# rlog58/dags-vae-search

Hardware: AMD Instinct MI355X
Metric: DAGs/sec VAE+predictor train step, n=12 batch 4096 per GPU, at 1 MI355X (higher is better)
Workload: dtype f32 (fwd bf16x6, bwd bf16x3 split products, fp32 accumulate); 1 GPU; synthetic_v12 DAGs (n=12, card=12, N=15 tokens), PACE-VAE train step: pack + fwd + bwd + clip_grad_norm_(1.0) + Adam(1e-4), train mode dropout 0.15; per_gpu_batch=4096, global_batch=4096, waves_per_workgroup=8, parallelism=single

## Files before the change

dags_vae_search_amd/_lib.py:

```python
from __future__ import annotations

import ctypes
import os
from ctypes import (POINTER, Structure, c_char, c_char_p, c_float, c_int, c_int32, c_int64, c_size_t, c_uint32,
                    c_uint64, c_void_p)

_HERE = os.path.dirname(os.path.abspath(__file__))
LIB_NAME = "libdvs_hip.so"

D_MODEL, HEADS, LAYERS, LATENT, FC_HIDDEN, EMB = 64, 8, 3, 32, 32, 32
MAX_TOKENS = 48
TILE_TOKENS = 16
DECODE_STATE_BYTES = 440
CLIP_SCRATCH_FLOATS = 4096
RECORD_BYTES = 96
LOSS_FLOATS = 5
ABI_VERSION = 202
GP_ACQ_MAX_INDUCING = 1023
STRUCT_HASH_INVALID = 0x7FFFFFFFFFFFFFFF
GEN_LABELS_CHOICE, GEN_ACCEPT_ISOLATES, GEN_ACCEPT_NO_CONNECTIVITY, GEN_GROUP_SHIFT = 1, 2, 4, 8
SCORE_TYPES = {"loglik": 0, "aic": 1, "bic": 2, "bde": 3, "bds": 4, "k2": 5, "bdj": 6}


class DvsShape(Structure):
# ... 21 lines not shown
    lib.dvs_record_bytes.argtypes = [P(DvsShape)]
    lib.dvs_pack_features.restype = c_int
    lib.dvs_pack_features.argtypes = [P(DvsShape), c_void_p, c_void_p, c_void_p, c_void_p, c_void_p, c_size_t, c_void_p,
                                      c_void_p]
    lib.dvs_build_records.restype = c_int
    lib.dvs_build_records.argtypes = [P(DvsShape), c_void_p, c_void_p, c_void_p, c_size_t, c_void_p, c_void_p]
    lib.dvs_loss_forward.restype = c_int
    lib.dvs_loss_forward.argtypes = [P(DvsShape), c_void_p, c_size_t, c_void_p, c_int64, c_void_p, c_size_t, c_void_p,
                                     c_void_p, c_void_p, c_void_p, c_void_p, c_void_p]
    lib.dvs_loss_forward_notify.restype = c_int
    lib.dvs_loss_forward_notify.argtypes = [P(DvsShape), c_void_p, c_size_t, c_void_p, c_int64, c_void_p, c_size_t, c_void_p,
                                            c_void_p, c_void_p, c_void_p, c_void_p, c_void_p, ctypes.c_uint32, c_void_p]
    lib.dvs_loss_backward.restype = c_int
    lib.dvs_loss_backward.argtypes = [P(DvsShape), c_void_p, c_size_t, c_void_p, c_int64, c_void_p, c_size_t, c_void_p,
                                      c_void_p, c_void_p]
    lib.dvs_loss_backward_sq.restype = c_int
    lib.dvs_loss_backward_sq.argtypes = [P(DvsShape), c_void_p, c_size_t, c_void_p, c_int64, c_void_p, c_size_t, c_void_p,
                                         c_void_p, c_void_p, c_void_p]
    lib.dvs_encode.restype = c_int
    lib.dvs_encode.argtypes = [P(DvsShape), c_void_p, c_size_t, c_void_p, c_int64, c_void_p, c_size_t, c_void_p, c_void_p,
                               c_void_p]
    lib.dvs_decode.restype = c_int
    lib.dvs_decode.argtypes = [P(DvsShape), c_void_p, c_int64, c_void_p, c_size_t, c_void_p, c_size_t, c_void_p, c_void_p,
                               c_void_p, c_size_t, c_void_p]
    lib.dvs_match_decoded.restype = c_int
    lib.dvs_match_decoded.argtypes = [c_int32, c_int32, c_int32, c_int32, c_int32, c_void_p, c_void_p, c_void_p, c_size_t,
                                      c_int32, c_void_p, c_void_p]
    lib.dvs_decoded_structures.restype = c_int
    lib.dvs_decoded_structures.argtypes = [c_int32, c_int32, c_int32, c_void_p, c_size_t, c_uint64, c_void_p, c_void_p,
                                           c_void_p, c_void_p, c_size_t, c_void_p, c_void_p]
    lib.dvs_structset_filter.restype = c_int
    lib.dvs_structset_filter.argtypes = [c_int32, c_int32, c_void_p, c_void_p, c_void_p, c_size_t, c_void_p, c_int32,
                                         c_void_p, c_void_p, c_size_t, c_void_p, c_void_p]
    lib.dvs_generate_dags.restype = c_int
    lib.dvs_generate_dags.argtypes = [c_int32, c_int32, c_int32, c_int32, c_void_p, c_uint64, c_int64, c_int32, c_int32,
                                      c_void_p, c_void_p, c_size_t, c_void_p, c_void_p]
    lib.dvs_generate_edge_counts.restype = c_int
    lib.dvs_generate_edge_counts.argtypes = [c_int32, c_int32, c_void_p, c_void_p, c_uint64, c_int64, c_void_p, c_void_p]
    lib.dvs_debug_launch.restype = c_int
    lib.dvs_debug_launch.argtypes = [c_size_t, c_void_p]
    lib.dvs_bic_scores.restype = c_int
    lib.dvs_bic_scores.argtypes = [c_int32, c_int32, c_int32, c_void_p, c_void_p, c_void_p, c_void_p, c_void_p, c_void_p,
                                   c_void_p]
    lib.dvs_bn_scores.restype = c_int
    lib.dvs_bn_scores.argtypes = [c_int32, c_int32, c_int32, c_void_p, c_void_p, c_void_p, c_int32, ctypes.c_double, c_void_p,
                                  c_void_p, c_void_p, c_void_p]
    lib.dvs_bn_toggle_scores.restype = c_int
    lib.dvs_bn_toggle_scores.argtypes = [c_int32, c_int32, c_int32, c_void_p, c_void_p, c_void_p, c_int32, ctypes.c_double,
                                         c_void_p, c_void_p, c_size_t, c_void_p, c_size_t, c_void_p, c_void_p]
    lib.dvs_hc_step.restype = c_int
    lib.dvs_hc_step.argtypes = [c_int32, c_int32, c_void_p, c_void_p, c_void_p, c_size_t, c_int32, ctypes.c_double, c_void_p,
                                c_int32, c_void_p, c_void_p, c_void_p, c_void_p, c_void_p, c_size_t, c_void_p, c_void_p]
    lib.dvs_tabu_step.restype = c_int
    lib.dvs_tabu_step.argtypes = lib.dvs_hc_step.argtypes[:-1] + [c_int32, c_void_p, c_size_t, c_void_p, c_int32, c_void_p,
                                                                  c_void_p, c_void_p, c_size_t, c_void_p]
    lib.dvs_hc_perturb.restype = c_int
    lib.dvs_hc_perturb.argtypes = [c_int32, c_int32, c_void_p, c_void_p, c_void_p, c_size_t, c_int32, c_void_p, c_void_p,
                                   c_void_p, c_uint64, c_uint32, c_void_p]
    lib.dvs_bic_parent_masks.restype = c_int
    lib.dvs_bic_parent_masks.argtypes = [c_int32, c_int32, c_int32, c_void_p, c_void_p, c_void_p, c_void_p, c_void_p]
    lib.dvs_gp_predict.restype = c_int
    lib.dvs_gp_predict.argtypes = [c_int32, c_int32, c_int32, c_void_p, c_void_p, c_void_p, ctypes.c_double, ctypes.c_double,
                                   ctypes.c_double, c_void_p, c_void_p]
    lib.dvs_gp_kernel.restype = c_int
    lib.dvs_gp_kernel.argtypes = [c_int32, c_int32, c_int32, c_void_p, c_void_p, ctypes.c_double, ctypes.c_double, c_void_p,
                                  c_void_p]
    lib.dvs_gp_kernel_backward.restype = c_int
    lib.dvs_gp_kernel_backward.argtypes = [c_int32, c_int32, c_int32, c_int32, c_void_p, c_void_p, ctypes.c_double,
                                           ctypes.c_double, c_void_p, c_void_p, c_void_p, c_void_p]
    lib.dvs_gp_acquire.restype = c_int
    lib.dvs_gp_acquire.argtypes = [c_int32, c_int32, c_int32, c_int32, c_void_p, c_void_p, c_void_p] + [ctypes.c_double] * 6 + \
        [c_void_p, c_void_p, c_void_p, c_void_p, c_void_p]
    lib.dvs_clip_adam.restype = c_int
    lib.dvs_clip_adam.argtypes = [c_int64, c_void_p, c_void_p, c_void_p, c_void_p, c_float, c_float, c_float, c_float,
                                  c_int64, c_float, c_void_p, c_void_p, c_void_p]
    lib.dvs_clip_adam_from_partials.restype = c_int
    lib.dvs_clip_adam_from_partials.argtypes = lib.dvs_clip_adam.argtypes
    lib.dvs_profile_enable.restype = None
    lib.dvs_profile_enable.argtypes = [c_int]
    lib.dvs_profile_collect.restype = c_int
    lib.dvs_profile_collect.argtypes = [c_void_p, c_int, c_void_p, c_void_p, c_int]
    lib.dvs_debug_activation.restype = c_int
    lib.dvs_debug_activation.argtypes = [P(DvsShape), c_void_p, c_int, c_void_p, c_void_p]
    return lib


EXPORTS = ["dvs_version", "dvs_last_error", "dvs_device_cus", "dvs_param_count", "dvs_param_table",
           "dvs_workspace_bytes", "dvs_record_bytes", "dvs_pack_features", "dvs_build_records", "dvs_loss_forward", "dvs_loss_forward_notify", "dvs_loss_backward", "dvs_loss_backward_sq", "dvs_encode", "dvs_decode", "dvs_match_decoded", "dvs_decoded_structures", "dvs_structset_filter", "dvs_generate_dags", "dvs_generate_edge_counts", "dvs_bic_scores", "dvs_bn_scores", "dvs_bn_toggle_scores", "dvs_hc_step", "dvs_tabu_step", "dvs_hc_perturb", "dvs_bic_parent_masks", "dvs_gp_predict", "dvs_gp_kernel", "dvs_gp_kernel_backward", "dvs_gp_acquire",
           "dvs_clip_adam", "dvs_clip_adam_from_partials", "dvs_debug_activation", "dvs_debug_launch", "dvs_profile_enable", "dvs_profile_collect"]


def profile_collect(lib):
    cap, stride = 64, 64
    names = ctypes.create_string_buffer(cap * stride)
    counts = (c_int * cap)()
    ms = (c_float * cap)()
    n = lib.dvs_profile_collect(names, stride, counts, ms, cap)
    out = {}
    for i in range(min(n, cap)):
        out[names.raw[i * stride:(i + 1) * stride].split(b"\0")[0].decode()] = (int(counts[i]), float(ms[i]))
    return out

_lib = None


def lib_path() -> str:
    return os.path.join(_HERE, LIB_NAME)


def load() -> ctypes.CDLL:
    global _lib
    if _lib is None:
        path = lib_path()
        if not os.path.exists(path):
            raise RuntimeError(
                f"{LIB_NAME} not found at {path}: build it with `python -c 'import __graft_entry__ as g; g.build()'` "
                f"(hipcc --offload-arch=gfx950).  dags_vae_search_amd has no CPU fallback.")
        _lib = bind(ctypes.CDLL(path))
        if _lib.dvs_version() != ABI_VERSION:
            raise RuntimeError(f"{LIB_NAME}: unexpected ABI version {_lib.dvs_version()}")
    return _lib


def check(lib, code: int, what: str):
    if code != 0:
        msg = lib.dvs_last_error()
        raise RuntimeError(f"{what} failed with code {code}: {msg.decode() if msg else ''}")


def make_shape(batch: int, n_tokens: int, n_classes: int, training: bool = False, dropout: float = 0.15,
               beta: float = 0.005, eps_scale: float = 0.01, dag_offset: int = 0, seed: int = 0) -> DvsShape:
    return DvsShape(int(batch), int(n_tokens), int(n_classes), 1 if training else 0, float(dropout), float(beta),
                    float(eps_scale), int(dag_offset) & 0xFFFFFFFF, int(seed) & 0xFFFFFFFFFFFFFFFF)


def record_bytes(lib, shape: DvsShape) -> int:
    n = int(lib.dvs_record_bytes(ctypes.byref(shape)))
    if n == 0:
        check(lib, 1, "dvs_record_bytes")
    return n


def is_wide(n_tokens: int, n_classes: int) -> bool:
    return n_tokens > TILE_TOKENS or n_classes > 16


def param_table(lib, shape: DvsShape):
    entries = (DvsParamEntry * 128)()
    n = lib.dvs_param_table(ctypes.byref(shape), entries, 128)
    if n <= 0:
        check(lib, 1, "dvs_param_table")
    table = []
    for e in entries[:n]:
        shp = (e.rows, e.cols) if e.cols else (e.rows,)
        table.append((e.name.decode(), int(e.offset), shp))
    total = int(lib.dvs_param_count(ctypes.byref(shape)))
    return table, total
```

dags_vae_search_amd/csrc/dvs_api.hip:

```cpp
#include <math.h>
#include <stdarg.h>
#include <stdio.h>
#include <stdlib.h>
#include <string.h>

#include "dvs_kernels.h"
#include "dvs_backward.h"
#include "dvs_wide.h"
#include "dvs_wimg.h"
#include "dvs_decode.h"

static thread_local char g_err[256] = "";

#include <map>
#include <mutex>
#include <string>
#include <utility>
#include <vector>
namespace {
struct ProfRec {
    const char* name;
#ifndef DVS_EMU
    hipEvent_t a, b;
#endif
};
std::mutex g_prof_mu;
bool g_prof_on = false;
std::vector<ProfRec> g_prof;
thread_local int t_prof_slot = -1;
}

void dvs_prof_begin(const char* name, dvs_stream_t st) {
    t_prof_slot = -1;
    std::lock_guard<std::mutex> lock(g_prof_mu);
    if (!g_prof_on) return;
    ProfRec r;
    r.name = name;
#ifndef DVS_EMU
    if (hipEventCreate(&r.a) != hipSuccess) return;
    if (hipEventCreate(&r.b) != hipSuccess) {
        (void)hipEventDestroy(r.a);
        return;
    }
    (void)hipEventRecord(r.a, st);
#endif
    t_prof_slot = (int)g_prof.size();
    g_prof.push_back(r);
}
void dvs_prof_end(dvs_stream_t st) {
    if (t_prof_slot < 0) return;
    std::lock_guard<std::mutex> lock(g_prof_mu);
#ifndef DVS_EMU
    if (t_prof_slot < (int)g_prof.size()) (void)hipEventRecord(g_prof[t_prof_slot].b, st);
#endif
    t_prof_slot = -1;
}
extern "C" void dvs_profile_enable(int on) {
    std::lock_guard<std::mutex> lock(g_prof_mu);
    g_prof_on = on != 0;
}
extern "C" int dvs_profile_collect(char* names, int name_stride, int* counts, float* total_ms, int cap) {
    std::map<std::string, std::pair<int, float>> agg;
    std::lock_guard<std::mutex> lock(g_prof_mu);
    for (auto& r : g_prof) {
        float ms = 0.f;
#ifndef DVS_EMU
        (void)hipEventSynchronize(r.b);
        (void)hipEventElapsedTime(&ms, r.a, r.b);
        (void)hipEventDestroy(r.a);
        (void)hipEventDestroy(r.b);
#endif
        auto& e = agg[r.name];
        e.first += 1;
        e.second += ms;
    }
    g_prof.clear();
    int i = 0;
    for (auto& kv : agg) {
        if (i >= cap) break;
        snprintf(names + (size_t)i * name_stride, name_stride, "%s", kv.first.c_str());
        counts[i] = kv.second.first;
        total_ms[i] = kv.second.second;
        ++i;
    }
    return (int)agg.size();
}

static int fail(int code, const char* msg) {
    snprintf(g_err, sizeof(g_err), "%s", msg);
    return code;
}

static thread_local int t_hip_err = 0;
// ... 142 lines not shown
    w.logvar = take((size_t)B * 32);
    w.z = take((size_t)B * 32);
    w.epsv = take((size_t)B * 32);
    w.mem = take(tile);
    w.dag_loss = take((size_t)B * 2);
    w.gA = take(tile);
    w.gB = take(tile);
    w.gq = take(tile);
    w.gk = take(tile);
    w.gv = take(tile);
    w.gmem = take(tile);
    w.genc = take(tile);
    w.gz = take((size_t)B * 64);
    w.nslab = nslab;
    w.slabs = take((size_t)nslab * (size_t)P);
    w.fcpart = take((size_t)DVS_FC_PARTS * (size_t)P);
    w.wimg = take((DVS_WIMG_BF16 + 1) / 2);
    w.limg = take(DvsLatImg::floats(NT));
    for (int blk = 0; blk < 9; ++blk) w.qkv[blk] = take(wide ? (size_t)B * NT * 12 * 256 : 0);
    w.total_floats = off;
    return w;
}

static int check_shape(const dvs_shape* s) {
    if (!s) return fail(1, "dvs: null shape");
    if (s->batch <= 0) return fail(2, "dvs: batch must be > 0");
    if (s->n_tokens < 4 || s->n_tokens > DVS_WTOK)
        return fail(3, "dvs: n_tokens (= max_num_vertices + 3) must be in [4, 48] in this build");
    if (s->n_classes < 4 || s->n_classes > DVS_WTOK)
        return fail(4, "dvs: n_classes (= vertex_label_cardinality + 3) must be in [4, 48] in this build");
    if (!(s->dropout >= 0.f && s->dropout < 1.f)) return fail(5, "dvs: dropout must be in [0, 1)");
    return 0;
}

static bool is_wide(const dvs_shape* s) { return s->n_tokens > DVS_MAXTOK || s->n_classes > 16; }
static int tiles_of(const dvs_shape* s) { return (s->n_tokens + 15) / 16; }
static size_t record_size(bool wide) { return wide ? sizeof(DvsRecordW) : sizeof(DvsRecord); }

static DvsDims make_dims(const dvs_shape* s) {
    DvsDims d;
    d.NT = tiles_of(s);
    d.B = s->batch;
    d.N = s->n_tokens;
    d.C = s->n_classes;
    d.training = s->training ? 1 : 0;
    d.drop.thr16 = (uint32_t)lrintf(s->dropout * 65536.0f);
    d.drop.on = (d.training && d.drop.thr16 > 0) ? 1 : 0;
    d.drop.scale = 1.0f / (1.0f - (float)d.drop.thr16 / 65536.0f);
    d.seed_lo = (uint32_t)(s->seed & 0xFFFFFFFFull);
    d.seed_hi = (uint32_t)(s->seed >> 32);
    d.dag_offset = s->dag_offset;
    d.beta = s->beta;
    d.eps_scale = s->eps_scale;
    d.debug = 0;
    return d;
}

static int num_slabs() {
    const int cus = dvs_device_cus();
    return cus > 0 ? cus : 256;
}
static int grid_for(int units, int per_wg, int cap) {
    const int want = (units + per_wg - 1) / per_wg;
    return want < cap ? want : cap;
}

static int waves_per_wg(const DvsDims& d, bool wide, int nslab) {
    const char* env = getenv("DVS_WAVES_PER_WG");
    const int force = env ? atoi(env) : 0;
    if (wide) return 8;
    if (force == 4 || force == 8) return force;
    return d.B <= 4 * nslab ? 4 : 8;
}
static int active_slabs(const DvsDims& d, bool wide, int nslab) {
    if (wide) return nslab;
    const int want = (d.B + 3) / 4;
    return want < nslab ? want : nslab;
}

static bool env_on(const char* name) {
    const char* v = getenv(name);
    return v && atoi(v) != 0;
}
static bool split_stack() {
    static const bool on = env_on("DVS_SPLIT_STACK");
    return on;
}
static bool latent_kernels_off() {
    static const bool on = env_on("DVS_LATENT_KERNELS");
    return on;
}
static bool latent_in_chain(bool chain, int nw) { return chain && !latent_kernels_off() && nw == 8; }

struct FwdGrids {
    int chain;
    int tiles16;
    int tiles8;
    int tiles4;
    int dags;
    int dags2;
    int dec4;
};

struct Step {
    DvsDims d;
    DvsLayout L;
    DvsWorkspace W;
    bool wide;
    const float* P;
    float* ws;
    const DvsRecord* rec;
    dvs_stream_t st;
    int nw;
    FwdGrids g;
    int slabs;
};
static Step make_step(const dvs_shape* s, const void* records, const float* params, void* workspace, void* stream) {
    Step c;
    c.d = make_dims(s);
    c.L = dvs_make_layout(c.d.N, c.d.C, nullptr, 0, nullptr);
    c.wide = is_wide(s);
    const int nslab = num_slabs();
    c.W = dvs_make_workspace(c.d.B, c.d.NT, c.L.total, nslab, c.wide);
    c.P = params;
    c.ws = (float*)workspace;
    c.rec = (const DvsRecord*)records;
    c.st = (dvs_stream_t)stream;
    c.nw = waves_per_wg(c.d, c.wide, nslab);
    const int tiles = c.d.B * c.d.NT;
    c.g.chain = grid_for(tiles, c.nw, nslab);
    c.g.tiles16 = grid_for(tiles, 16, nslab);
    c.g.tiles8 = grid_for(tiles, 8, nslab);
    c.g.tiles4 = grid_for(tiles, 4, nslab);
    c.g.dags = grid_for(c.d.B, 1, nslab);
    c.g.dags2 = c.d.B < 2 * c.g.dags ? c.d.B : 2 * c.g.dags;
    c.g.dec4 = grid_for(c.d.B, 4, nslab);
    c.slabs = active_slabs(c.d, c.wide, nslab);
    return c;
}

static int check_records(const char* fn, size_t records_bytes, int batch, bool wide) {
    const size_t need = (size_t)batch * record_size(wide);
    if (records_bytes >= need) return 0;
    char msg[240];
    snprintf(msg, sizeof(msg), "%s: records_bytes %zu < batch * dvs_record_bytes = %zu", fn, records_bytes, need);
    return fail(14, msg);
}
static int check_buffers(const Step& c, const char* fn, size_t records_bytes, int64_t n_params, size_t workspace_bytes) {
    if (int e = check_records(fn, records_bytes, c.d.B, c.wide)) return e;
    char msg[240];
    if (n_params < c.L.total) {
        snprintf(msg, sizeof(msg), "%s: n_params %lld < dvs_param_count = %lld", fn, (long long)n_params, (long long)c.L.total);
        return fail(14, msg);
    }
    const size_t need = c.W.total_floats * sizeof(float);
    if (workspace_bytes < need) {
        snprintf(msg, sizeof(msg), "%s: workspace_bytes %zu < dvs_workspace_bytes = %zu", fn, workspace_bytes, need);
        return fail(14, msg);
    }
    return 0;
}

extern "C" int64_t dvs_param_count(const dvs_shape* s) {
    if (check_shape(s)) return -1;
    return dvs_make_layout(s->n_tokens, s->n_classes, nullptr, 0, nullptr).total;
}

extern "C" int dvs_param_table(const dvs_shape* s, dvs_param_entry* out, int cap) {
    if (check_shape(s)) return -1;
    int count = 0;
    dvs_make_layout(s->n_tokens, s->n_classes, out, cap, &count);
    return count;
}

extern "C" size_t dvs_workspace_bytes(const dvs_shape* s) {
// ... 194 lines not shown
    auto add = [&](int64_t src, size_t dst, int rows, int flags) {
        DvsImgJob& j = J.job[J.count++];
        j.src = src;
        j.dst = (int64_t)dst;
        j.rows = rows;
        j.flags = flags;
    };
    auto attn = [&](const DvsAttnP& p, int block) {
        const size_t b = img_attn(block);
        add(p.in_w, b + DvsAttnImg::Win, 192, wide ? 0 : 2);
        add(p.out_w, b + DvsAttnImg::Wout, 64, wide ? 0 : 4);
        add(p.out_w, b + DvsAttnImg::WoutT, 64, 1 | (wide ? 0 : 4));
        add(p.in_w, b + DvsAttnImg::WinB, 192, 16 | (wide ? 0 : 2));
        for (int q = 0; q < 3; ++q)
            add(p.in_w + 4096 * q, b + DvsAttnImg::WinT + (size_t)q * 2 * DVS_IMG64, 64, 1 | (wide ? 0 : 2));
    };
    auto ffn = [&](const DvsFfnP& p, int block) {
        const size_t b = img_ffn(block);
        add(p.l1_w, b + DvsFfnImg::W1, 64, 0);
        add(p.l2_w, b + DvsFfnImg::W2, 64, 0);
        add(p.l2_w, b + DvsFfnImg::W2T, 64, 1);
        add(p.l1_w, b + DvsFfnImg::W1T, 64, 1);
    };
    for (int i = 0; i < DVS_LAYERS; ++i) {
        attn(L.enc[i].sa, blk_enc_attn(i));
        ffn(L.enc[i].ff, blk_enc_ffn(i));
        attn(L.dec[i].sa, blk_dec_self(i));
        attn(L.dec[i].ca, blk_dec_cross(i));
        ffn(L.dec[i].ff, blk_dec_ffn(i));
    }
    if (!wide) {
        add(L.edge0_w, DVS_WIMG_LOSS + DvsLossImg::Wa, 64, 8);
        add(L.edge0_w + 64, DVS_WIMG_LOSS + DvsLossImg::Wb, 64, 8);
        add(L.edge0_w, DVS_WIMG_LOSS + DvsLossImg::WaT, 64, 8 | 1);
        add(L.edge0_w + 64, DVS_WIMG_LOSS + DvsLossImg::WbT, 64, 8 | 1);
    }
    dvs_bf16* wimg = (dvs_bf16*)(c.ws + c.W.wimg);
    DvsLatImgArgs lat;
    lat.fc1_w = c.P + L.fc1_w;
    lat.fc2_w = c.P + L.fc2_w;
    lat.fc3_w = c.P + L.fc3_w;
    lat.fc3_b = c.P + L.fc3_b;
    lat.img = c.ws + c.W.limg;
    lat.N = c.d.N;
    lat.NT = c.d.NT;
    DvsLossHeadArgs head;
    memset(&head, 0, sizeof(head));
    if (!wide) {
        head_params(c, head);
        head.ln_g = c.P + L.dec[DVS_LAYERS - 1].n3.w;
        head.ln_b = c.P + L.dec[DVS_LAYERS - 1].n3.b;
        head.dst = (float*)(wimg + DVS_WIMG_LOSS + DvsLossImg::Head);
        head.C = c.d.C;
        head.W1 = c.P + L.W1;
        head.W2 = c.P + L.W2;
        head.lab_w = c.P + L.lab_w;
        head.lab_b = c.P + L.lab_b;
        head.dst_emb = (float*)(wimg + DVS_WIMG_EMB);
        head.N = c.d.N;
    }
    dvs_launch_prepare_images(J, c.P, wimg, lat, head, c.st);
}

static void launch_embed_fwd(const Step& c, const EmbedArgs& e) {
    if (c.wide) dvs_launch_embed_fwd_w(e, c.g.tiles4, c.st);
    else if (c.nw == 4) dvs_launch_embed_fwd(e, c.g.chain, 4, c.st);
    else dvs_launch_embed_fwd(e, c.g.tiles16, 16, c.st);
}
static void launch_attn_fwd(const Step& c, const AttnArgs& a) {
    if (c.wide) dvs_launch_attn_fwd_w(a, c.g.dags, c.st);
    else if (c.nw == 4) dvs_launch_attn_fwd(a, c.g.chain, 4, c.st);
    else dvs_launch_attn_fwd(a, c.g.tiles8, 8, c.st);
}
static void launch_ffn_fwd(const Step& c, const FfnArgs& f) {
    if (c.nw == 4) dvs_launch_ffn_fwd(f, c.g.chain, 4, c.st);
    else dvs_launch_ffn_fwd(f, c.g.tiles16, 16, c.st);
}
static void launch_loss_fwd(const Step& c, const LossArgs& a) {
    if (c.wide) dvs_launch_loss_fwd_w(a, c.g.dags2, c.st);
    else if (c.nw == 4) dvs_launch_loss_fwd(a, c.g.chain, 4, c.st);
    else dvs_launch_loss_fwd(a, c.g.tiles8, 8, c.st);
}
struct FwdChain {
    FwdStackArgs stack;
    const Step& c;
    int tag;
    bool chain;
    FwdChain(const Step& step, int tag_) : c(step), tag(tag_), chain(!step.wide && !split_stack()) { memset(&stack, 0, sizeof(stack)); }
    FwdPhase& next(int kind) {
        if (stack.nphase == DVS_FWD_STACK_PHASES) flush();
        FwdPhase& ph = stack.ph[stack.nphase++];
        ph.kind = kind;
        return ph;
    }
    void attn(const AttnArgs& a) {
        if (chain) next(DVS_FPH_ATTN).u.a = a;
        else launch_attn_fwd(c, a);
    }
    void ffn(const FfnArgs& f) {
        if (chain) next(DVS_FPH_FFN).u.f = f;
        else launch_ffn_fwd(c, f);
    }
    bool latent(const LatentArgs& l) {
        if (!latent_in_chain(chain, c.nw) || stack.nphase == 0 || stack.nphase == DVS_FWD_STACK_PHASES) return false;
        next(DVS_FPH_LATENT).u.l = l;
        return true;
    }
    void flush() {
        if (stack.nphase > 0) dvs_launch_fwd_stack(stack, tag, c.g.chain, c.nw, c.st);
        stack.nphase = 0;
    }
};

static void encoder_forward(const Step& c, const LatentArgs& lat, bool dec_embed = false, bool save_qkv = false) {
    EmbedArgs e = embed_args(c, 0);
    e.out = c.ws + c.W.act[0];
    if (dec_embed) {
        e.out2 = c.ws + c.W.act[7];
        e.site2 = 2;
    }
    launch_embed_fwd(c, e);
    FwdChain chain(c, 0);
    const DvsNormP* norm = nullptr;
    int prev = 0;
    for (int i = 0; i < DVS_LAYERS; ++i) {
        const auto& pl = c.L.enc[i];
        const int sa = slot_enc(i, 0), sf = slot_enc(i, 1);
        AttnArgs a = attn_args(c, pl.sa, blk_enc_attn(i), prev, norm, nullptr, sa, site_enc(i, 0));
        if (!save_qkv) a.qkv = nullptr;
        chain.attn(a);
        FfnArgs f = ffn_args(c, pl.ff, blk_enc_ffn(i), sa, pl.n1, sf, site_enc(i, 2));
        if (i == DVS_LAYERS - 1) {
            f.out_norm = c.ws + c.W.enc_out;
            f.ng = c.P + pl.n2.w;
            f.nb = c.P + pl.n2.b;
        }
        chain.ffn(f);
        norm = &pl.n2;
        prev = sf;
    }
    const bool fused = chain.latent(lat);
    chain.flush();
    if (!fused) dvs_launch_latent_fwd(lat, c.st);
}

static void decoder_forward(const Step& c, int dec_in) {
    FwdChain chain(c, 1);
    const DvsNormP* norm = nullptr;
    int prev = dec_in;
    for (int i = 0; i < DVS_LAYERS; ++i) {
        const auto& pl = c.L.dec[i];
        const int s0 = slot_dec(i, 0), s1 = slot_dec(i, 1), s2 = slot_dec(i, 2);
        chain.attn(attn_args(c, pl.sa, blk_dec_self(i), prev, norm, nullptr, s0, site_dec(i, 0)));
        chain.attn(attn_args(c, pl.ca, blk_dec_cross(i), s0, &pl.n1, c.ws + c.W.mem, s1, site_dec(i, 2)));
        chain.ffn(ffn_args(c, pl.ff, blk_dec_ffn(i), s1, pl.n2, s2, site_dec(i, 4)));
        norm = &pl.n3;
        prev = s2;
    }
    chain.flush();
}

extern "C" int dvs_loss_forward(const dvs_shape* s, const void* records, size_t records_bytes, const float* params,
                                int64_t n_params, void* workspace, size_t workspace_bytes, const float* eps,
                                const int32_t* status, float* losses, float* mu, float* logvar, void* stream) {
    return dvs_loss_forward_notify(s, records, records_bytes, params, n_params, workspace, workspace_bytes, eps,
                                   (int32_t*)status, losses, mu, logvar, nullptr, 0u, stream);
}

extern "C" int dvs_loss_forward_notify(const dvs_shape* s, const void* records, size_t records_bytes, const float* params,
                                       int64_t n_params, void* workspace, size_t workspace_bytes, const float* eps,
                                       int32_t* status, float* losses, float* mu, float* logvar, void* host_tail,
                                       uint32_t host_seq, void* stream) {
    if (int e = check_shape(s)) return e;
    if (!records || !params || !workspace || !losses) return fail(10, "dvs_loss_forward: null pointer");
    const Step c = make_step(s, records, params, workspace, stream);
    if (int e = check_buffers(c, "dvs_loss_forward", records_bytes, n_params, workspace_bytes)) return e;
    call_begin();
    prepare_images(c);
    encoder_forward(c, latent_args(c, eps, true), c.d.drop.on, true);
    decoder_forward(c, c.d.drop.on ? 7 : 0);
    launch_loss_fwd(c, loss_args(c));
    FinalizeArgs fa;
    fa.B = c.d.B;
    fa.beta = c.d.beta;
    fa.dag_loss = c.ws + c.W.dag_loss;
    fa.status = status;
    fa.losses = losses;
    fa.host_tail = (float*)host_tail;
    fa.host_seq = host_seq;
    dvs_launch_finalize(fa, c.st);
    const size_t nb = (size_t)c.d.B * 32 * sizeof(float);
    if (mu) copy_out(mu, c.ws + c.W.mu, nb, c.st);
    if (logvar) copy_out(logvar, c.ws + c.W.logvar, nb, c.st);
    return call_end("dvs_loss_forward");
}

extern "C" int dvs_encode(const dvs_shape* s, const void* records, size_t records_bytes, const float* params,
                          int64_t n_params, void* workspace, size_t workspace_bytes, float* mu, float* logvar,
                          void* stream) {
    if (int e = check_shape(s)) return e;
    if (!records || !params || !workspace || !mu || !logvar) return fail(10, "dvs_encode: null pointer");
    const Step c = make_step(s, records, params, workspace, stream);
    if (int e = check_buffers(c, "dvs_encode", records_bytes, n_params, workspace_bytes)) return e;
    call_begin();
    prepare_images(c);
    LatentArgs la = latent_args(c, nullptr, false);
    la.dims.training = 0;
    encoder_forward(c, la);
    const size_t nb = (size_t)c.d.B * 32 * sizeof(float);
    copy_out(mu, c.ws + c.W.mu, nb, c.st);
    copy_out(logvar, c.ws + c.W.logvar, nb, c.st);
    return call_end("dvs_encode");
}

extern "C" int dvs_decode(const dvs_shape* s, const float* params, int64_t n_params, void* workspace,
                          size_t workspace_bytes, void* records, size_t records_bytes, const float* z,
                          const float* uniforms, void* state_out, size_t state_bytes, void* stream) {
    if (int e = check_shape(s)) return e;
    if (!params || !workspace || !records || !z || !state_out) return fail(10, "dvs_decode: null pointer");
    if (s->training) return fail(13, "dvs_decode: generation runs in eval mode (shape.training must be 0)");
    const Step c = make_step(s, records, params, workspace, stream);
    if (int e = check_buffers(c, "dvs_decode", records_bytes, n_params, workspace_bytes)) return e;
    if (state_bytes < (size_t)s->batch * sizeof(dvs_decode_state))
        return fail(14, "dvs_decode: state_bytes < batch * sizeof(dvs_decode_state)");
    call_begin();
    prepare_images(c);
    dvs_launch_decode_memory(c.d, z, c.P + c.L.fc3_w, c.P + c.L.fc3_b, c.ws + c.W.mem, c.st);
    DecodeArgs a;
    memset(&a, 0, sizeof(a));
    a.dims = c.d;
    a.wide = c.wide ? 1 : 0;
    a.rec = records;
    a.state = (DvsDecodeState*)state_out;
    head_input(c, a);
    a.uniforms = uniforms;
    dvs_launch_decode_init(a, c.st);
    EmbedArgs e = embed_args(c, 2);
    e.out = c.ws + c.W.act[7];
    for (int idx = 2; idx < c.d.N; ++idx) {
        launch_embed_fwd(c, e);
        decoder_forward(c, 7);
        a.idx = idx;
        dvs_launch_decode_step(a, c.g.dec4, c.st);
    }
    return call_end("dvs_decode");
}

extern "C" int dvs_match_decoded_impl(int B, int n, int card, int R, int wide, const uint8_t* labels, const void* preds,
                                      const void* states, int budget, uint8_t* flags, void* stream);
extern "C" int dvs_match_decoded(int32_t batch, int32_t n_vars, int32_t card, int32_t repeats, int32_t preds_are_u64,
                                 const uint8_t* labels, const void* preds, const void* states, size_t state_bytes,
                                 int32_t budget, uint8_t* flags, void* stream) {
    if (batch <= 0 || repeats <= 0) return fail(2, "dvs_match_decoded: batch and repeats must be > 0");
    if ((int64_t)batch * repeats > (int64_t)1 << 30) return fail(2, "dvs_match_decoded: batch * repeats must be <= 2^30");
    if (n_vars < 1 || n_vars > 45) return fail(3, "dvs_match_decoded: n_vars must be in [1, 45]");
    if (card < 1 || card > 45) return fail(3, "dvs_match_decoded: card must be in [1, 45]");
    if (!preds_are_u64 && n_vars > 16) return fail(12, "dvs_match_decoded: 16-bit predecessor rows hold at most 16 vertices");
    if (budget < 1) return fail(12, "dvs_match_decoded: budget must be >= 1");
    if (!labels || !preds || !states || !flags) return fail(10, "dvs_match_decoded: null pointer");
    const size_t need = (size_t)batch * repeats * sizeof(dvs_decode_state);
    if (state_bytes < need) {
        char msg[160];
        snprintf(msg, sizeof(msg), "dvs_match_decoded: state_bytes < batch * repeats * DVS_DECODE_STATE_BYTES = %zu", need);
        return fail(14, msg);
    }
    call_begin();
    if (int e = dvs_match_decoded_impl(batch, n_vars, card, repeats, preds_are_u64 ? 1 : 0, labels, preds, states, budget,
                                       flags, stream))
        return e;
    return call_end("dvs_match_decoded");
}

extern "C" int dvs_decoded_structures_impl(int B, int n, int wide, const void* states, uint64_t hash_mask, uint8_t* flags,
                                           uint8_t* labels, void* preds, uint64_t* keys, uint64_t* hashes, void* stream);
extern "C" int dvs_structset_filter_impl(int B, int n, const uint64_t* sorted_hashes, const int64_t* order,
                                         const uint64_t* keys, const uint8_t* flags, int S, const uint64_t* seen_hashes,
                                         const uint64_t* seen_keys, uint8_t* out, void* stream);
static int fail_size(const char* what, size_t need) {
    char msg[200];
    snprintf(msg, sizeof(msg), "%s = %zu", what, need);
    return fail(14, msg);
}
extern "C" int dvs_decoded_structures(int32_t batch, int32_t n_vars, int32_t preds_are_u64, const void* states,
                                      size_t state_bytes, uint64_t hash_mask, uint8_t* flags, uint8_t* labels, void* preds,
                                      uint64_t* keys, size_t keys_bytes, uint64_t* hashes, void* stream) {
    if (batch <= 0) return fail(2, "dvs_decoded_structures: batch must be > 0");
    if (batch > 1 << 30) return fail(2, "dvs_decoded_structures: batch must be <= 2^30");
    if (n_vars < 1 || n_vars > 45) return fail(3, "dvs_decoded_structures: n_vars must be in [1, 45]");
    if (!preds_are_u64 && n_vars > 16) return fail(12, "dvs_decoded_structures: 16-bit predecessor rows hold at most 16 vertices");
    if (!states || !flags || !labels || !preds || !keys || !hashes) return fail(10, "dvs_decoded_structures: null pointer");
    if (state_bytes < (size_t)batch * sizeof(dvs_decode_state))
        return fail_size("dvs_decoded_structures: state_bytes < batch * DVS_DECODE_STATE_BYTES", (size_t)batch * sizeof(dvs_decode_state));
    if (keys_bytes < (size_t)batch * n_vars * 8)
        return fail_size("dvs_decoded_structures: keys_bytes < batch * n_vars * 8", (size_t)batch * n_vars * 8);
    call_begin();
    if (int e = dvs_decoded_structures_impl(batch, n_vars, preds_are_u64 ? 1 : 0, states, hash_mask, flags, labels, preds, keys,
                                            hashes, stream))
        return e;
    return call_end("dvs_decoded_structures");
}

extern "C" int dvs_structset_filter(int32_t batch, int32_t n_vars, const uint64_t* sorted_hashes, const int64_t* order,
                                    const uint64_t* keys, size_t keys_bytes, const uint8_t* flags, int32_t seen_count,
                                    const uint64_t* seen_hashes, const uint64_t* seen_keys, size_t seen_keys_bytes,
                                    uint8_t* out, void* stream) {
    if (batch < 0 || seen_count < 0) return fail(2, "dvs_structset_filter: batch and seen_count must be >= 0");
    if (batch > 1 << 30) return fail(2, "dvs_structset_filter: batch must be <= 2^30");
    if (n_vars < 1 || n_vars > 45) return fail(3, "dvs_structset_filter: n_vars must be in [1, 45]");
    if (batch == 0) return 0;
    if (!sorted_hashes || !order || !keys || !flags || !out) return fail(10, "dvs_structset_filter: null pointer");
    if (seen_count > 0 && (!seen_hashes || !seen_keys)) return fail(10, "dvs_structset_filter: null pointer (seen set)");
    if (keys_bytes < (size_t)batch * n_vars * 8)
        return fail_size("dvs_structset_filter: keys_bytes < batch * n_vars * 8", (size_t)batch * n_vars * 8);
    if (seen_keys_bytes < (size_t)seen_count * n_vars * 8)
        return fail_size("dvs_structset_filter: seen_keys_bytes < seen_count * n_vars * 8", (size_t)seen_count * n_vars * 8);
    call_begin();
    if (int e = dvs_structset_filter_impl(batch, n_vars, sorted_hashes, order, keys, flags, seen_count, seen_hashes, seen_keys,
                                          out, stream))
        return e;
    return call_end("dvs_structset_filter");
}

extern "C" int dvs_generate_dags_impl(int B, int n, int card, int wide, const int* num_edges, uint64_t seed, uint32_t dag_offset,
                                      int try_limit, int flags, int gshift, uint8_t* labels, void* preds, int* attempts,
// ... 332 lines not shown
```

dags_vae_search_amd/csrc/dvs_api_backward.inc:

```

static AttnBwdArgs attn_bwd_args(const Step& c, const DvsAttnP& ap, int block, int in, const DvsNormP* norm, const float* kv,
                                 const float* gpre, int site0) {
    AttnBwdArgs a;
    memset(&a, 0, sizeof(a));
    a.wimg = wimg_attn(c, block);
    a.dims = c.d;
    a.rec = c.rec;
    a.xin = c.ws + c.W.act[in];
    a.ln = ln_of(c, in, norm);
    a.kv = kv;
    a.in_w = c.P + ap.in_w;
    a.in_b = c.P + ap.in_b;
    a.out_w = c.P + ap.out_w;
    a.out_b = c.P + ap.out_b;
    a.gpre = gpre;
    a.gq = c.ws + c.W.gq;
    a.gk = c.ws + c.W.gk;
    a.gv = c.ws + c.W.gv;
    a.site_prob = site0;
    a.site_post = site0 + 1;
    a.slab = c.ws + c.W.slabs;
    a.P = c.L.total;
    a.o_out_w = ap.out_w;
    a.o_out_b = ap.out_b;
// ... 6 lines not shown
    ProjBwdArgs a;
    memset(&a, 0, sizeof(a));
    a.dims = c.d;
    a.xin = c.ws + c.W.act[in];
    a.ln = ln_of(c, in, norm);
    a.w = c.P + ap.in_w;
    a.wimg = (const dvs_bf16*)wimg_attn(c, block) + DvsAttnImg::WinT;
    a.gy[0] = c.ws + c.W.gq;
    a.gy[1] = c.ws + c.W.gk;
    a.gy[2] = c.ws + c.W.gv;
    a.gres = gres;
    a.gout = gout;
    a.slot_order = c.wide ? 0 : 1;
    a.slab = c.ws + c.W.slabs;
    a.P = c.L.total;
    a.o_w = ap.in_w;
    a.o_b = ap.in_b;
    a.o_ln_g = norm ? norm->w : -1;
    a.o_ln_b = norm ? norm->b : -1;
    return a;
}

static FfnBwdArgs ffn_bwd_args(const Step& c, const DvsFfnP& fp, int block, int in, const DvsNormP& norm, const float* gpre,
                               float* gout, int site0) {
    FfnBwdArgs a;
    memset(&a, 0, sizeof(a));
    a.dims = c.d;
    a.xin = c.ws + c.W.act[in];
    a.ln = ln_of(c, in, &norm);
    a.l1_w = c.P + fp.l1_w;
    a.l1_b = c.P + fp.l1_b;
    a.l2_w = c.P + fp.l2_w;
    a.l2_b = c.P + fp.l2_b;
    a.wimg = wimg_ffn(c, block);
    a.gpre = gpre;
    a.gout = gout;
    a.site_hidden = site0;
    a.site_post = site0 + 1;
    a.slab = c.ws + c.W.slabs;
    a.P = c.L.total;
    a.o_l1_w = fp.l1_w;
    a.o_l1_b = fp.l1_b;
    a.o_l2_w = fp.l2_w;
    a.o_l2_b = fp.l2_b;
    a.o_ln_g = norm.w;
    a.o_ln_b = norm.b;
    a.o_own_g = -1;
    a.o_own_b = -1;
    return a;
}

extern "C" int dvs_loss_backward(const dvs_shape* s, const void* records, size_t records_bytes, const float* params,
                                 int64_t n_params, void* workspace, size_t workspace_bytes, const float* gcoef,
                                 float* grads, void* stream) {
    return dvs_loss_backward_sq(s, records, records_bytes, params, n_params, workspace, workspace_bytes, gcoef, grads, nullptr,
                                stream);
}

extern "C" int dvs_loss_backward_sq(const dvs_shape* s, const void* records, size_t records_bytes, const float* params,
                                    int64_t n_params, void* workspace, size_t workspace_bytes, const float* gcoef,
                                    float* grads, float* clip_scratch, void* stream) {
    if (int e = check_shape(s)) return e;
    if (!records || !params || !workspace || !gcoef || !grads) return fail(10, "dvs_loss_backward: null pointer");
    const Step c = make_step(s, records, params, workspace, stream);
    if (int e = check_buffers(c, "dvs_loss_backward", records_bytes, n_params, workspace_bytes)) return e;
    if (clip_scratch && 2 + dvs_sq_parts(c.L.total) > DVS_CLIP_SCRATCH_FLOATS)
        return fail(14, "dvs_loss_backward_sq: clip_scratch (DVS_CLIP_SCRATCH_FLOATS) is too small for this parameter count");
    call_begin();
    const DvsLayout& L = c.L;
    const DvsWorkspace& W = c.W;
    float* ws = c.ws;
    dvs_stream_t st = c.st;
    const bool wide = c.wide;
    const int grid = c.slabs;
    const int nw = c.nw;
    const bool chain = !wide && !split_stack();
    const bool chain_local = wide && !split_stack();
    BwdStackArgs stack;
    memset(&stack, 0, sizeof(stack));
    int stack_tag = 0;
    auto flush_stack = [&]() {
        if (stack.nphase > 0) dvs_launch_bwd_stack(stack, stack_tag, grid, nw, st);
        stack.nphase = 0;
        stack.has_latent = 0;
    };
    auto next_phase = [&](int kind) -> BwdPhase& {
        if (stack.nphase == DVS_STACK_PHASES) flush_stack();
        BwdPhase& ph = stack.ph[stack.nphase++];
        ph.kind = kind;
        return ph;
    };
    auto launch_ffn_bwd = [&](const FfnBwdArgs& f) {
        if (chain || chain_local) next_phase(DVS_PH_FFN).u.f = f;
        else dvs_launch_ffn_bwd(f, grid, nw, st);
    };
    auto launch_attn_bwd = [&](const AttnBwdArgs& a) {
        if (chain) {
            next_phase(DVS_PH_ATTN).u.a = a;
        } else if (wide) {
            flush_stack();
            dvs_launch_attn_bwd_w(a, grid, st);
        } else {
            dvs_launch_attn_bwd(a, grid, nw, st);
        }
    };
    auto launch_proj_bwd = [&](const ProjBwdArgs& a) {
        if (chain || chain_local) next_phase(DVS_PH_PROJ1 + 2).u.p = a;
        else dvs_launch_proj_bwd(a, 3, grid, nw, st);
    };

    float* cur = ws + W.gA;
    float* oth = ws + W.gB;
    {
        LossArgs la = loss_args(c);
        la.gcoef = gcoef;
        la.gout = cur;
        la.slab = ws + W.slabs;
        la.P = L.total;
        la.o_node0_w = L.node0_w;
        la.o_node0_b = L.node0_b;
        la.o_node2_w = L.node2_w;
        la.o_node2_b = L.node2_b;
        la.o_edge0_w = L.edge0_w;
        la.o_edge0_b = L.edge0_b;
        la.o_edge2_w = L.edge2_w;
        la.o_edge2_b = L.edge2_b;
        la.o_ln_g = L.dec[DVS_LAYERS - 1].n3.w;
        la.o_ln_b = L.dec[DVS_LAYERS - 1].n3.b;
        if (wide) dvs_launch_loss_bwd_w(la, grid, st);
        else dvs_launch_loss_bwd(la, grid, st);
    }
    const int dec_in = c.d.drop.on ? 7 : 0;
    for (int i = DVS_LAYERS - 1; i >= 0; --i) {
        const auto& pl = L.dec[i];
        const int s0 = slot_dec(i, 0), s1 = slot_dec(i, 1);
        launch_ffn_bwd(ffn_bwd_args(c, pl.ff, blk_dec_ffn(i), s1, pl.n2, cur, oth, site_dec(i, 4)));
        std::swap(cur, oth);
        launch_attn_bwd(attn_bwd_args(c, pl.ca, blk_dec_cross(i), s0, &pl.n1, ws + W.mem, cur, site_dec(i, 2)));
        ProjBwdArgs pq = proj_bwd_args(c, pl.ca, blk_dec_cross(i), s0, &pl.n1, cur, oth);
        pq.xin2 = ws + W.mem;
        pq.gout2 = ws + W.gmem;
        pq.accumulate_out2 = i != DVS_LAYERS - 1;
        launch_proj_bwd(pq);
        std::swap(cur, oth);
        const int sp = i > 0 ? slot_dec(i - 1, 2) : dec_in;
        const DvsNormP* np = i > 0 ? &L.dec[i - 1].n3 : nullptr;
        launch_attn_bwd(attn_bwd_args(c, pl.sa, blk_dec_self(i), sp, np, nullptr, cur, site_dec(i, 0)));
        launch_proj_bwd(proj_bwd_args(c, pl.sa, blk_dec_self(i), sp, np, cur, oth));
        std::swap(cur, oth);
    }
    flush_stack();
    stack_tag = 1;
    float* gdec_emb = cur;
    float* freebuf = oth;

    const bool fc_deferred = latent_in_chain(chain, nw);
    FcDwArgs fcdw;
    {
        LatentBwdArgs a;
        memset(&a, 0, sizeof(a));
        a.dims = c.d;
        a.gmem = ws + W.gmem;
        a.mu = ws + W.mu;
        a.logvar = ws + W.logvar;
        a.epsv = ws + W.epsv;
        a.limg = ws + W.limg;
        a.gcoef = gcoef;
        a.gz = ws + W.gz;
        a.genc = ws + W.genc;
        if (fc_deferred) {
            stack.has_latent = 1;
            stack.lat = a;
        } else {
            dvs_launch_latent_bwd(a, st);
        }
        FcDwArgs& f = fcdw;
        memset(&f, 0, sizeof(f));
        f.dims = c.d;
        f.gz = ws + W.gz;
        f.xenc = ws + W.enc_out;
        f.gmem = ws + W.gmem;
        f.z = ws + W.z;
        f.fcpart = ws + W.fcpart;
        f.P = L.total;
        f.o_fc1_w = L.fc1_w;
        f.o_fc1_b = L.fc1_b;
        f.o_fc2_w = L.fc2_w;
        f.o_fc2_b = L.fc2_b;
        f.o_fc3_w = L.fc3_w;
        f.o_fc3_b = L.fc3_b;
        if (!fc_deferred) dvs_launch_fc_dw(f, st);
    }
    cur = ws + W.genc;
    oth = freebuf;
    for (int i = DVS_LAYERS - 1; i >= 0; --i) {
        const auto& pl = L.enc[i];
        const int s0 = slot_enc(i, 0), s1 = slot_enc(i, 1);
        FfnBwdArgs f = ffn_bwd_args(c, pl.ff, blk_enc_ffn(i), s0, pl.n1, cur, oth, site_enc(i, 2));
        if (i == DVS_LAYERS - 1) {
            f.own_pre = ws + W.act[s1];
            f.own = ln_of(c, s1, &pl.n2);
            f.o_own_g = pl.n2.w;
            f.o_own_b = pl.n2.b;
        }
        launch_ffn_bwd(f);
        std::swap(cur, oth);
        const int sp = i > 0 ? slot_enc(i - 1, 1) : 0;
        const DvsNormP* np = i > 0 ? &L.enc[i - 1].n2 : nullptr;
        launch_attn_bwd(attn_bwd_args(c, pl.sa, blk_enc_attn(i), sp, np, nullptr, cur, site_enc(i, 0)));
        launch_proj_bwd(proj_bwd_args(c, pl.sa, blk_enc_attn(i), sp, np, cur, oth));
        std::swap(cur, oth);
    }
    flush_stack();
    if (fc_deferred) dvs_launch_fc_dw(fcdw, st);
    {
        EmbedArgs e = embed_args(c, 0);
        e.gout = cur;
        e.slab = ws + W.slabs;
        e.P = L.total;
        e.oW1 = L.W1;
        e.oW2 = L.W2;
        e.olab_w = L.lab_w;
        e.olab_b = L.lab_b;
        if (wide) dvs_launch_embed_bwd_w(e, gdec_emb, 2, grid, st);
        else dvs_launch_embed_bwd(e, gdec_emb, 2, grid, nw, st);
    }
    ReduceArgs r;
    r.slab = ws + W.slabs;
    r.fcpart = ws + W.fcpart;
    r.grads = grads;
    r.P = L.total;
    r.nslab = grid;
    r.fc_lo1 = L.fc1_w;
    r.fc_hi1 = L.dec[0].sa.in_w;
    r.fc_lo2 = L.fc3_w;
    r.fc_hi2 = L.total;
    r.sqpart = clip_scratch ? clip_scratch + 2 : nullptr;
    dvs_launch_reduce_slabs(r, st);
    return call_end("dvs_loss_backward");
}

extern "C" int dvs_clip_adam(int64_t n, float* params, float* grads, float* exp_avg, float* exp_avg_sq, float lr,
                             float beta1, float beta2, float adam_eps, int64_t step, float max_norm, float* scratch,
                             const float* guard, void* stream) {
    if (n <= 0 || !params || !grads || !exp_avg || !exp_avg_sq || !scratch) return fail(10, "dvs_clip_adam: bad argument");
    if (step < 1) return fail(12, "dvs_clip_adam: step is 1-based");
    call_begin();
    dvs_launch_clip_adam(n, params, grads, exp_avg, exp_avg_sq, lr, beta1, beta2, adam_eps, step, max_norm, scratch, guard, false,
                         (dvs_stream_t)stream);
    return call_end("dvs_clip_adam");
}

extern "C" int dvs_clip_adam_from_partials(int64_t n, float* params, float* grads, float* exp_avg, float* exp_avg_sq, float lr,
                                           float beta1, float beta2, float adam_eps, int64_t step, float max_norm,
                                           float* scratch, const float* guard, void* stream) {
    if (n <= 0 || !params || !grads || !exp_avg || !exp_avg_sq || !scratch) return fail(10, "dvs_clip_adam_from_partials: bad argument");
    if (step < 1) return fail(12, "dvs_clip_adam_from_partials: step is 1-based");
    if (2 + dvs_sq_parts(n) > DVS_CLIP_SCRATCH_FLOATS) return fail(14, "dvs_clip_adam_from_partials: more partials than the scratch holds");
    call_begin();
    dvs_launch_clip_adam(n, params, grads, exp_avg, exp_avg_sq, lr, beta1, beta2, adam_eps, step, max_norm, scratch, guard, true,
                         (dvs_stream_t)stream);
    return call_end("dvs_clip_adam_from_partials");
}
```

dags_vae_search_amd/csrc/dvs_backward.h:

```cpp
#pragma once
#include "dvs_kernels.h"
#include "dvs_stage.h"

struct FfnBwdArgs {
    DvsDims dims;
    const float* xin;
    DvsLN ln;
    const float *l1_w, *l1_b, *l2_w, *l2_b;
    const void* wimg;
    const float* gpre;
    const float* own_pre;
    DvsLN own;
    float* gout;
    int site_hidden, site_post;
    float* slab;
    int64_t P;
    int64_t o_l1_w, o_l1_b, o_l2_w, o_l2_b, o_ln_g, o_ln_b, o_own_g, o_own_b;
};

struct ProjBwdArgs {
    DvsDims dims;
    const float* xin;
    DvsLN ln;
    const float* w;
    const void* wimg;
    const float* gy[3];
    const float* gres;
    float* gout;
    int accumulate_out;
    int slot_order;
    const float* xin2;
    float* gout2;
    int accumulate_out2;
    float* slab;
    int64_t P;
    int64_t o_w, o_b, o_ln_g, o_ln_b;
};

struct AttnBwdArgs {
    DvsDims dims;
    const DvsRecord* rec;
    const float* xin;
    DvsLN ln;
    const float* kv;
    const float *in_w, *in_b, *out_w, *out_b;
    const void* wimg;
    const float* gpre;
    float *gq, *gk, *gv;
    int site_prob, site_post;
    float* slab;
    int64_t P;
    int64_t o_out_w, o_out_b;
    const float* qkv;
};

struct LatentBwdArgs {
    DvsDims dims;
    const float* gmem;
    const float *mu, *logvar, *epsv;
    const float* limg;
    const float* gcoef;
    float* gz;
    float* genc;
};

struct FcDwArgs {
    DvsDims dims;
    const float* gz;
    const float* xenc;
    const float* gmem;
    const float* z;
    float* fcpart;
    int64_t P;
    int64_t o_fc1_w, o_fc1_b, o_fc2_w, o_fc2_b, o_fc3_w, o_fc3_b;
};

struct ReduceArgs {
    const float* slab;
    const float* fcpart;
    float* grads;
    int64_t P;
    int nslab;
    int64_t fc_lo1, fc_hi1, fc_lo2, fc_hi2;
    float* sqpart;
};

enum { DVS_PH_FFN = 0, DVS_PH_ATTN = 1, DVS_PH_PROJ1 = 2, DVS_PH_PROJ2 = 3, DVS_PH_PROJ3 = 4 };
#define DVS_STACK_PHASES 9
struct BwdPhase {
    int kind, pad;
    union {
        FfnBwdArgs f;
        AttnBwdArgs a;
        ProjBwdArgs p;
    } u;
};
struct BwdStackArgs {
    int nphase;
    int has_latent;
    BwdPhase ph[DVS_STACK_PHASES];
    DvsStagePlan plan[DVS_STACK_PHASES];
    LatentBwdArgs lat;
};
static_assert(sizeof(BwdStackArgs) <= 4096, "kernel argument block limit");
void dvs_launch_bwd_stack(const BwdStackArgs& s, int tag, int grid, int nw, dvs_stream_t st);
void dvs_launch_ffn_bwd(const FfnBwdArgs& a, int grid, int nw, dvs_stream_t st);
void dvs_launch_proj_bwd(const ProjBwdArgs& a, int nproj, int grid, int nw, dvs_stream_t st);
void dvs_launch_attn_bwd(const AttnBwdArgs& a, int grid, int nw, dvs_stream_t st);
void dvs_launch_loss_bwd(const LossArgs& a, int grid, dvs_stream_t st);
void dvs_launch_embed_bwd(const EmbedArgs& a, const float* gout2, int site2, int grid, int nw, dvs_stream_t st);
void dvs_launch_latent_bwd(const LatentBwdArgs& a, dvs_stream_t st);
void dvs_launch_fc_dw(const FcDwArgs& a, dvs_stream_t st);
void dvs_launch_reduce_slabs(const ReduceArgs& a, dvs_stream_t st);
void dvs_launch_clip_adam(int64_t n, float* params, float* grads, float* m, float* v, float lr, float b1, float b2,
                          float eps, int64_t step, float max_norm, float* scratch, const float* guard, bool have_partials,
                          dvs_stream_t st);
inline int dvs_sq_parts(int64_t n) { return (int)(((n + 3) / 4 + 63) / 64); }

template <int OT, int IT>
__device__ __forceinline__ void dvs_stage_dw(float* region, const f4 (&dw)[OT][IT], const Lane& L) {
    constexpr int COLS = 16 * IT;
    float* mine = region + L.wave * (256 * OT * IT);
#pragma unroll
    for (int ot = 0; ot < OT; ++ot)
#pragma unroll
        for (int it = 0; it < IT; ++it)
#pragma unroll
            for (int reg = 0; reg < 4; ++reg) mine[(16 * ot + 4 * L.g + reg) * COLS + 16 * it + L.r] = dw[ot][it][reg];
}
template <int OT, int IT>
__device__ __forceinline__ void dvs_flush_dw(const float* region, float* dst, const Lane& L, int rows = 16 * OT,
                                             int ld_dst = 16 * IT, int cols_used = 16 * IT, bool rperm = false,
                                             bool cperm = false) {
    constexpr int COLS = 16 * IT, SZ = 256 * OT * IT;
    if (cperm) {
        for (int i = dvs_tid(); i < rows * COLS; i += blockDim.x) {
            float s = region[i];
            for (int w = 1; w < L.nwaves; ++w) s += region[w * SZ + i];
            const int row = i / COLS, col = i - row * COLS;
            dst[(size_t)(rperm ? dvs_pi(row) : row) * ld_dst + (cperm ? dvs_pi(col) : col)] = s;
        }
        return;
    }
    if (cols_used == COLS && (ld_dst & 3) == 0) {
        for (int i = dvs_tid() * 4; i < rows * COLS; i += blockDim.x * 4) {
            f4 s = *(const f4*)(region + i);
            for (int w = 1; w < L.nwaves; ++w) s += *(const f4*)(region + w * SZ + i);
            const int row = i / COLS, col = i - row * COLS;
            *(f4*)(dst + (size_t)(rperm ? dvs_pi(row) : row) * ld_dst + col) = s;
        }
        return;
    }
    for (int i = dvs_tid(); i < rows * COLS; i += blockDim.x) {
        float s = region[i];
        for (int w = 1; w < L.nwaves; ++w) s += region[w * SZ + i];
        const int row = i / COLS, col = i - row * COLS;
        if (col < cols_used) dst[(size_t)row * ld_dst + col] = s;
    }
}
template <int NT>
__device__ __forceinline__ void dvs_stage_vec(float* region, const f4 (&v)[NT], float* scr, const Lane& L) {
#pragma unroll
    for (int t = 0; t < NT; ++t) *(f4*)(scr + L.r * DVS_LD + 16 * t + 4 * L.g) = v[t];
    dvs_wave_sync();
    if (L.lane < 16 * NT) {
        float s = 0.f;
#pragma unroll
        for (int rr = 0; rr < 16; ++rr) s += scr[rr * DVS_LD + L.lane];
        region[L.wave * (16 * NT) + L.lane] = s;
    }
    dvs_wave_sync();
}
template <int NT>
__device__ __forceinline__ void dvs_flush_vec(const float* region, float* dst, const Lane& L, int n = 16 * NT,
                                              bool perm = false) {
    for (int i = dvs_tid(); i < n; i += blockDim.x) {
        float s = region[i];
        for (int w = 1; w < L.nwaves; ++w) s += region[w * (16 * NT) + i];
        dst[perm ? dvs_pi(i) : i] = s;
    }
}
constexpr int DVS_RED_MAT = 4 * 4096;
constexpr int DVS_RED_VEC = 4 * 64;

__device__ __forceinline__ void dvs_ln_bwd(f4 (&dx)[4], const f4 (&xhat)[4], float rstd, const float* lg, f4 (&dgam)[4],
                                           f4 (&dbet)[4], const Lane& L) {
    float s1 = 0.f, s2 = 0.f;
#pragma unroll
// ... 101 lines not shown
```

dags_vae_search_amd/csrc/dvs_bwd_phases.h:

```cpp
#pragma once
#include "dvs_backward.h"
#include "dvs_wimg.h"

constexpr int DVS_PROJB_SLOT = 6 * DVS_PKB;
static size_t projb_lds_bytes(int nproj) {
    return (size_t)2 * nproj * 64 * DVS_LDB * sizeof(dvs_bf16) + 128 * 4 + (size_t)8 * DVS_PROJB_SLOT * sizeof(dvs_bf16) + 64;
}


#include "dvs_stage.h"

constexpr size_t DVS_BWD_EPI_FLOOR = 80 * 1024;
static_assert(8 * DVS_IMG64 * sizeof(dvs_bf16) + (192 + 64 + 128) * 4 + 16 <= DVS_BWD_EPI_FLOOR, "attention-core plan");
static_assert(7 * DVS_IMG64 * sizeof(dvs_bf16) + 6 * 64 * 4 + 16 <= DVS_BWD_EPI_FLOOR, "FFN plan");
static_assert(6 * DVS_IMG64 * sizeof(dvs_bf16) + 128 * 4 + 16 <= DVS_BWD_EPI_FLOOR, "projection plan");
static_assert(DVS_BWD_EPI_FLOOR + (2 * 4096 + 8 * 6 * 64) * 4 <= 7 * DVS_IMG64 * sizeof(dvs_bf16) + (6 * 64 + 8 * 2 * DVS_SCR) * 4, "FFN");
static_assert(DVS_BWD_EPI_FLOOR + (4096 + 8 * 64) * 4 <= 8 * DVS_IMG64 * sizeof(dvs_bf16) + (384 + 8 * 2 * DVS_SCR) * 4, "attention core");
static_assert(DVS_BWD_EPI_FLOOR + (1 * 4096 + 8 * 3 * 64) * 4 <= 2 * DVS_IMG64 * sizeof(dvs_bf16) + 8 * DVS_PROJB_SLOT * sizeof(dvs_bf16), "1 projection");
static_assert(DVS_BWD_EPI_FLOOR + (3 * 4096 + 8 * 5 * 64) * 4 <= 6 * DVS_IMG64 * sizeof(dvs_bf16) + 8 * DVS_PROJB_SLOT * sizeof(dvs_bf16), "3 projections");
__device__ __forceinline__ float* dvs_bwd_epi(char* smem) { return (float*)(smem + DVS_BWD_EPI_FLOOR); }

#ifdef DVS_STAMPS
DVS_STAMP_DECL(dvs_stamps_bwd);
#endif
// ... 54 lines not shown
struct ProjBLds {
    dvs_bf16* WT;
    float *lg, *lb;
    dvs_bf16* slots;
    int* gcount;
};
DVS_HD inline ProjBLds projb_lds(char* smem, int nproj) {
    ProjBLds l;
    l.WT = (dvs_bf16*)smem;
    l.lg = (float*)(l.WT + nproj * 2 * DVS_IMG64);
    l.lb = l.lg + 64;
    l.gcount = (int*)(l.lb + 64);
    l.slots = (dvs_bf16*)(l.gcount + 4);
    return l;
}

inline void ffnb_plan(DvsStagePlan& p, const FfnBwdArgs& a, char* smem) {
    const FfnBLds l = ffnb_lds(smem);
    dvs_plan_clear(p);
    dvs_plan_seg(p, smem, l.W2Th, (const dvs_bf16*)a.wimg + DvsFfnImg::W2T, (int)(7 * DVS_IMG64));
    dvs_plan_vec(p, smem, l.b1, a.l1_b, 64);
    dvs_plan_vec(p, smem, l.b2, a.l2_b, 64);
    dvs_plan_vec(p, smem, l.lg, a.ln.g, a.ln.stats ? 64 : 0);
    dvs_plan_vec(p, smem, l.lb, a.ln.b, a.ln.stats ? 64 : 0);
    dvs_plan_vec(p, smem, l.og, a.own.g, a.own_pre ? 64 : 0);
    dvs_plan_vec(p, smem, l.ob, a.own.b, a.own_pre ? 64 : 0);
    p.zero_int = (int)(((const char*)l.gcount - smem) >> 2);
    dvs_plan_cold(p, a.xin, a.own_pre, a.dims.B * a.dims.NT);
    dvs_plan_seal(p);
}
inline void attnb_plan(DvsStagePlan& p, const AttnBwdArgs& a, char* smem) {
    const AttnBLds l = attnb_lds(smem);
    dvs_plan_clear(p);
    dvs_plan_seg(p, smem, l.WoTh, (const dvs_bf16*)a.wimg + DvsAttnImg::WoutT, (int)(8 * DVS_IMG64));
    dvs_plan_vec(p, smem, l.inb, a.in_b, 192, true);
    dvs_plan_vec(p, smem, l.outb, a.out_b, 64);
    dvs_plan_vec(p, smem, l.lg, a.ln.g, a.ln.stats ? 64 : 0);
    dvs_plan_vec(p, smem, l.lb, a.ln.b, a.ln.stats ? 64 : 0);
    p.zero_int = (int)(((const char*)l.gcount - smem) >> 2);
    dvs_plan_cold(p, a.xin, a.kv, a.dims.B * a.dims.NT);
    dvs_plan_seal(p);
}
inline void projb_plan(DvsStagePlan& p, const ProjBwdArgs& a, int nproj, char* smem) {
    const ProjBLds l = projb_lds(smem, nproj);
    dvs_plan_clear(p);
    dvs_plan_seg(p, smem, l.WT, a.wimg, (int)(nproj * 2 * DVS_IMG64));
    dvs_plan_vec(p, smem, l.lg, a.ln.g, a.ln.stats ? 64 : 0);
    dvs_plan_vec(p, smem, l.lb, a.ln.b, a.ln.stats ? 64 : 0);
    p.zero_int = (int)(((const char*)l.gcount - smem) >> 2);
    dvs_plan_cold(p, a.xin, a.xin2, a.dims.B * a.dims.NT);
    dvs_plan_seal(p);
}
inline void dvs_bwd_plan(DvsStagePlan& p, const BwdPhase& ph, char* smem) {
    switch (ph.kind) {
        case DVS_PH_FFN: ffnb_plan(p, ph.u.f, smem); break;
        case DVS_PH_ATTN: attnb_plan(p, ph.u.a, smem); break;
        case DVS_PH_PROJ1: projb_plan(p, ph.u.p, 1, smem); break;
        case DVS_PH_PROJ2: projb_plan(p, ph.u.p, 2, smem); break;
        default: projb_plan(p, ph.u.p, 3, smem); break;
    }
}
struct DvsBwdTail {
    DvsPrefetch<DVS_PF_BWD_TAIL> pf;
};
template <class PP>
__device__ __forceinline__ void dvs_tail_issue(DvsBwdTail& t, PP next, bool has_next) {
    if (has_next && dvs_tid() < DVS_PF_THREADS) dvs_prefetch_issue<false>(t.pf, next, dvs_tid(), DVS_PF_THREADS);
}
template <class PP>
__device__ __forceinline__ void dvs_tail_commit(const DvsBwdTail& t, PP next, bool has_next, char* smem) {
    if (has_next && dvs_tid() < DVS_PF_THREADS) dvs_prefetch_commit<false>(t.pf, next, smem, dvs_tid(), DVS_PF_THREADS);
}
template <class PP>
__device__ __forceinline__ void dvs_bwd_tail_end(const DvsBwdTail& tail, const DvsTouch& touch, PP mine, PP next, bool has_next,
                                                 char* smem) {
    DVS_STAMP(dvs_stamps_bwd, mine, 5);
    dvs_tail_commit(tail, next, has_next, smem);
    DVS_STAMP(dvs_stamps_bwd, mine, 6);
    dvs_touch_done(touch);
}

template <int NW, class PP>
__device__ __forceinline__ void dvs_ffn_bwd_phase(const FfnBwdArgs& a, char* smem, PP mine, bool stage_mine, PP next,
                                                  bool has_next) {
    const FfnBLds l = ffnb_lds(smem);
    DVS_STAMP(dvs_stamps_bwd, mine, 0);
    if (stage_mine) {
        dvs_stage_now<(NW == 8 ? DVS_PF_BWD : DVS_PF_BWD_TAIL)>(mine, smem);
        __syncthreads();
    }
    DVS_STAMP(dvs_stamps_bwd, mine, 1);
    int* gcount = l.gcount;
    const Lane L = dvs_lane();
    const DvsDrop D = dvs_drop_of(a.dims);
    const int B = a.dims.B * a.dims.NT;
    float* sA = l.slots + L.wave * 2 * DVS_SCR;
    float* sB = sA + DVS_SCR;
    DvsGroup G = {gcount + (L.wave >> 2), 0};
    f4 aW1[4] = {f4_zero(), f4_zero(), f4_zero(), f4_zero()}, aW2[4] = {f4_zero(), f4_zero(), f4_zero(), f4_zero()};
    f4 ab1 = f4_zero(), ab2 = f4_zero();
    float vgam = 0.f, vbet = 0.f, vog = 0.f, vob = 0.f;
    dvs_bf16* const bslots = (dvs_bf16*)l.slots;
    constexpr int BSTRIDE = 2 * 2 * DVS_SCR;
    bool gate = !stage_mine;
    for (int base = dvs_bid() * NW; base < B; base += gridDim.x * NW) {
        const int dag = base + L.wave;
        const bool live = dag < B;
        const size_t dg = live ? dag : 0;
        const DvsTile T = dvs_tile_of((int)dg, a.dims);
        const int N = T.Nl;
        const int Nl = live ? N : 0;
        f4 x[4], xhat[4], gp[4];
        float rstd;
        {
            DvsRawX rx;
            dvs_load_x_issue(rx, a.xin, a.ln, dg, L);
            DVS_PHASE_GATE(gate);
            dvs_load_tile(gp, a.gpre, dg, L);
            dvs_load_x_finish<true>(x, xhat, rstd, rx, a.ln, l.lg, l.lb, Nl, L);
            dvs_zero_rows(gp, Nl, L);
        }
        if (a.own_pre) {
            f4 po[4], pxh[4], t0[4];
            float prstd;
            dvs_load_x<true>(po, pxh, prstd, a.own_pre, a.own, l.og, l.ob, dg, Nl, L);
#pragma unroll
            for (int t = 0; t < 4; ++t) t0[t] = gp[t] * pxh[t];
            dvs_park_T(sA, t0, L);
            dvs_park_T(sB, gp, L);
            dvs_wave_sync();
            vog += dvs_colsum(sA, L);
            vob += dvs_colsum(sB, L);
            dvs_wave_sync();
            dvs_ln_bwd_core(gp, pxh, prstd, l.og, L);
        }
        const uint32_t gdag = a.dims.dag_offset + (uint32_t)T.dag;
        const uint32_t khid = dvs_site_key(a.dims.seed_lo, a.dims.seed_hi, a.site_hidden, gdag);
        const uint32_t kpost = dvs_site_key(a.dims.seed_lo, a.dims.seed_hi, a.site_post, gdag);
        f4 hpre[4], hd[4];
#pragma unroll
        for (int t = 0; t < 4; ++t) hpre[t] = dvs_vecT(l.b1, t, L);
        dvs_matb3<4>(hpre, dvs_split3_T(x), l.W1x6, 64, 0, L);
#pragma unroll
        for (int t = 0; t < 4; ++t)
#pragma unroll
            for (int kk = 0; kk < 4; ++kk) hd[t][kk] = (live && L.r < N) ? fmaxf(hpre[t][kk], 0.f) : 0.f;
        const uint32_t hid_bits = dvs_dropout_bits(khid, D, L, T.tok0);
        dvs_dropout_apply(hd, hid_bits, D);
        f4 dy[4];
#pragma unroll
        for (int t = 0; t < 4; ++t) dy[t] = gp[t];
        dvs_dropout_tile(dy, kpost, D, L, T.tok0);
        dvs_park_bf((dvs_bf16*)sA, dy, L);
        dvs_park_bf((dvs_bf16*)sB, hd, L);
        dvs_group_barrier(G, L);
        dvs_coop_dw_bf(aW2, ab2, bslots, bslots + 2 * DVS_SCR, BSTRIDE, L);
        f4 dh[4] = {f4_zero(), f4_zero(), f4_zero(), f4_zero()};
        dvs_matb_T<4>(dh, dvs_split_T(dy), l.W2Th, l.W2Tl, 0, L);
        dvs_dropout_apply(dh, hid_bits, D);
#pragma unroll
        for (int t = 0; t < 4; ++t)
#pragma unroll
            for (int kk = 0; kk < 4; ++kk) dh[t][kk] = hpre[t][kk] > 0.f ? dh[t][kk] : 0.f;
        dvs_group_barrier(G, L);
        dvs_park_bf((dvs_bf16*)sA, dh, L);
        dvs_park_bf((dvs_bf16*)sB, x, L);
        dvs_group_barrier(G, L);
        dvs_coop_dw_bf(aW1, ab1, bslots, bslots + 2 * DVS_SCR, BSTRIDE, L);
        f4 dx[4];
#pragma unroll
        for (int t = 0; t < 4; ++t) dx[t] = gp[t];
        dvs_matb_T<4>(dx, dvs_split_T(dh), l.W1Th, l.W1Tl, 0, L);
        dvs_group_barrier(G, L);
        if (a.ln.stats) {
            f4 t0[4];
#pragma unroll
            for (int t = 0; t < 4; ++t) t0[t] = dx[t] * xhat[t];
            dvs_park_T(sA, t0, L);
            dvs_park_T(sB, dx, L);
            dvs_wave_sync();
            vgam += dvs_colsum(sA, L);
            vbet += dvs_colsum(sB, L);
            dvs_wave_sync();
            dvs_ln_bwd_core(dx, xhat, rstd, l.lg, L);
        }
        if (live) dvs_store_tile(a.gout, dag, dx, L);
        if (base == dvs_bid() * NW) DVS_STAMP(dvs_stamps_bwd, mine, 7);
    }
    DVS_PHASE_GATE(gate);
    DvsBwdTail tail;
    DVS_STAMP(dvs_stamps_bwd, mine, 2);
    dvs_tail_issue(tail, next, has_next);
    const DvsTouch touch = dvs_touch_first(next, has_next, NW, L.wave, L.lane);
    DVS_STAMP(dvs_stamps_bwd, mine, 3);
    dvs_lds_barrier();
    DVS_STAMP(dvs_stamps_bwd, mine, 4);
    float* slab = a.slab + (size_t)dvs_bid() * a.P;
    float* const buf1 = dvs_bwd_epi(smem);
    float* const buf2 = buf1 + 4096;
    float* red = buf2 + 4096;
    dvs_coop_stage<NW>(buf1, aW1, L);
    dvs_coop_stage<NW>(buf2, aW2, L);
    red[(L.wave * 6 + 0) * 64 + L.lane] = 0.f;
    red[(L.wave * 6 + 1) * 64 + L.lane] = 0.f;
    red[(L.wave * 6 + 2) * 64 + L.lane] = vgam;
    red[(L.wave * 6 + 3) * 64 + L.lane] = vbet;
    red[(L.wave * 6 + 4) * 64 + L.lane] = vog;
    red[(L.wave * 6 + 5) * 64 + L.lane] = vob;
    dvs_wave_sync();
    if (L.r == 0) {
#pragma unroll
        for (int reg = 0; reg < 4; ++reg) {
            red[(L.wave * 6 + 0) * 64 + 16 * (L.wave & 3) + 4 * L.g + reg] = ab1[reg];
            red[(L.wave * 6 + 1) * 64 + 16 * (L.wave & 3) + 4 * L.g + reg] = ab2[reg];
        }
    }
    dvs_lds_barrier();
    dvs_coop_flush<NW>(buf1, slab + a.o_l1_w, aW1, L);
    dvs_coop_flush<NW>(buf2, slab + a.o_l2_w, aW2, L);
    for (int k = dvs_tid() >> 6; k < 6; k += NW) {
        const int f = dvs_tid() & 63;
// ... 122 lines not shown
    dvs_lds_barrier();
    DVS_STAMP(dvs_stamps_bwd, mine, 4);
    float* slab = a.slab + (size_t)dvs_bid() * a.P;
    const bool so = a.slot_order != 0;
    float* const bufs = dvs_bwd_epi(smem);
#pragma unroll
    for (int p = 0; p < NPROJ; ++p) dvs_coop_stage<NW>(bufs + 4096 * p, aW[p], L);
    float* red = bufs + 4096 * NPROJ;
#pragma unroll
    for (int p = 0; p < NPROJ; ++p) red[(L.wave * (NPROJ + 2) + p) * 64 + L.lane] = 0.f;
    red[(L.wave * (NPROJ + 2) + NPROJ) * 64 + L.lane] = vgam;
    red[(L.wave * (NPROJ + 2) + NPROJ + 1) * 64 + L.lane] = vbet;
    dvs_wave_sync();
    if (L.r == 0) {
#pragma unroll
        for (int p = 0; p < NPROJ; ++p)
#pragma unroll
            for (int reg = 0; reg < 4; ++reg) red[(L.wave * (NPROJ + 2) + p) * 64 + 16 * (L.wave & 3) + 4 * L.g + reg] = ab[p][reg];
    }
    dvs_lds_barrier();
#pragma unroll
    for (int p = 0; p < NPROJ; ++p) dvs_coop_flush<NW>(bufs + 4096 * p, slab + a.o_w + 4096 * p, aW[p], L, so, false);
    for (int k = dvs_tid() >> 6; k < NPROJ + 2; k += NW) {
        const int f = dvs_tid() & 63;
        float s = 0.f;
        for (int w = 0; w < NW; ++w) s += red[(w * (NPROJ + 2) + k) * 64 + f];
        if (k < NPROJ) slab[a.o_b + 64 * k + (so ? dvs_pi(f) : f)] = s;
        else if (a.o_ln_g >= 0) slab[(k == NPROJ ? a.o_ln_g : a.o_ln_b) + f] = s;
    }
    dvs_bwd_tail_end(tail, touch, mine, next, has_next, smem);
}


__device__ __forceinline__ float dvs_bit_select(uint32_t bits, int pos, float v) {
#ifndef DVS_EMU
    const uint32_t m = (uint32_t)__builtin_amdgcn_sbfe((int)bits, pos, 1);
#else
    const uint32_t m = ((bits >> pos) & 1u) ? 0xFFFFFFFFu : 0u;
#endif
    return __uint_as_float(__float_as_uint(v) & m);
}
struct ProbMask {
    uint32_t T;
    uint32_t S[4];
};
__device__ __forceinline__ ProbMask dvs_prob_mask(uint32_t key, const DvsDrop& D, const Lane& L) {
    ProbMask m;
    m.T = 0xFFFFFFFFu;
    if (D.on) {
        uint32_t bits = 0;
#pragma unroll
        for (int h = 0; h < 8; ++h) {
            const uint32_t p0 = (uint32_t)((h * 16 + L.r) * 8 + 2 * L.g);
            const uint32_t h0 = dvs_draw(key, p0), h1 = dvs_draw(key, p0 + 1);
            bits |= ((h0 & 0xFFFFu) >= D.thr16 ? 1u : 0u) << (4 * h);
            bits |= ((h0 >> 16) >= D.thr16 ? 1u : 0u) << (4 * h + 1);
            bits |= ((h1 & 0xFFFFu) >= D.thr16 ? 1u : 0u) << (4 * h + 2);
            bits |= ((h1 >> 16) >= D.thr16 ? 1u : 0u) << (4 * h + 3);
        }
        m.T = bits;
    }
#pragma unroll
    for (int reg = 0; reg < 4; ++reg)
        m.S[reg] = D.on ? ((uint32_t)__shfl((int)m.T, 4 * L.g + reg + 16 * (L.r >> 2)) >> (L.r & 3)) : 0xFFFFFFFFu;
    return m;
}
__device__ __forceinline__ f4 mask_T(const ProbMask& m, int h, const DvsDrop& D) {
    if (!D.on) return f4_splat(1.f);
    f4 r;
#pragma unroll
    for (int reg = 0; reg < 4; ++reg) r[reg] = dvs_bit_select(m.T, 4 * h + reg, D.scale);
    return r;
}
__device__ __forceinline__ f4 mask_S(const ProbMask& m, int h, const DvsDrop& D) {
    if (!D.on) return f4_splat(1.f);
    f4 r;
#pragma unroll
    for (int reg = 0; reg < 4; ++reg) r[reg] = dvs_bit_select(m.S[reg], 4 * h, D.scale);
    return r;
}

template <int NW, class PP>
__device__ __forceinline__ void dvs_attn_bwd_phase(const AttnBwdArgs& a, char* smem, PP mine, bool stage_mine, PP next,
                                                   bool has_next) {
    const AttnBLds l = attnb_lds(smem);
    DVS_STAMP(dvs_stamps_bwd, mine, 0);
    if (stage_mine) {
        dvs_stage_now<(NW == 8 ? DVS_PF_BWD : DVS_PF_BWD_TAIL)>(mine, smem);
        __syncthreads();
    }
    DVS_STAMP(dvs_stamps_bwd, mine, 1);
    const Lane L = dvs_lane();
    const DvsDrop D = dvs_drop_of(a.dims);
    const int N = a.dims.N, B = a.dims.B;
    float* sA = l.slots + L.wave * 2 * DVS_SCR;
    float* sB = sA + DVS_SCR;
    float* st = l.stats + L.wave * DVS_ATTNB_TSCR;
    DvsGroup G = {l.gcount + (L.wave >> 2), 0};
    const float scale = 0.35355339059327373f;
    f4 aWo[4] = {f4_zero(), f4_zero(), f4_zero(), f4_zero()};
    f4 abo = f4_zero();
    bool gate = !stage_mine;
    DVS_PHASE_GATE(gate);
    for (int base = dvs_bid() * NW; base < B; base += gridDim.x * NW) {
        const int dag = base + L.wave;
        const bool live = dag < B;
        const size_t dg = live ? dag : 0;
        const int Nl = live ? N : 0;
        const uint32_t gdag = a.dims.dag_offset + (uint32_t)dg;
        const uint32_t kprob = dvs_site_key(a.dims.seed_lo, a.dims.seed_hi, a.site_prob, gdag);
        const unsigned allowed_r = live ? a.rec[dg].allowed[L.r] : (1u << L.r);
        f4 q[4], k[4], v[4];
        {
            f4 x[4], kv[4], dummy[4];
            float rstd;
            {
                dvs_load_x<false>(x, dummy, rstd, a.xin, a.ln, l.lg, l.lb, dg, Nl, L);
                if (a.kv) dvs_load_tile(kv, a.kv, dg, L);
            }
            if (!a.kv) {
#pragma unroll
                for (int t = 0; t < 4; ++t) kv[t] = x[t];
            }
#pragma unroll
            for (int t = 0; t < 4; ++t) {
                q[t] = dvs_vecT(l.inb, t, L);
                k[t] = dvs_vecT(l.inb + 64, t, L);
                v[t] = f4_splat(l.inb[128 + 16 * t + L.r]);
            }
            {
                const SplitT xs = dvs_split_T(x);
                dvs_matb_T<4>(q, xs, l.Winh, l.Winl, 0, L);
                if (a.kv) {
                    const SplitT ks = dvs_split_T(kv);
                    dvs_matb_T<4>(k, ks, l.Winh, l.Winl, 64, L);
                    dvs_matb_N<4>(v, ks, l.Winh, l.Winl, 128, L);
                } else {
                    dvs_matb_T<4>(k, xs, l.Winh, l.Winl, 64, L);
                    dvs_matb_N<4>(v, xs, l.Winh, l.Winl, 128, L);
                }
            }
#pragma unroll
            for (int t = 0; t < 4; ++t) q[t] *= scale;
        }
        f4 qN[4], kN[4], vT[4], dOT[4], dON[4];
        {
            f4 dy[4];
            dvs_load_grad(dy, a.gpre, dg, Nl, L);
            dvs_dropout_tile(dy, dvs_site_key(a.dims.seed_lo, a.dims.seed_hi, a.site_post, gdag), D, L);
            dvs_park_bf((dvs_bf16*)sA, dy, L);
#pragma unroll
            for (int t = 0; t < 4; ++t) dOT[t] = f4_zero();
            dvs_matb_T<4>(dOT, dvs_split_T(dy), l.WoTh, l.WoTl, 0, L);
        }
        dvs_t2n<4>(qN, q, sB, L);
        dvs_t2n<4>(kN, k, sB, L);
        dvs_n2t<4>(vT, v, sB, L);
        dvs_t2n<4>(dON, dOT, sB, L);

        const ProbMask pm = dvs_prob_mask(kprob, D, L);
        const bool hsel = ((L.r & 3) >> 1) != 0;
        bool ok[4];
        unsigned al4[4];
#pragma unroll
        for (int reg = 0; reg < 4; ++reg) {
            ok[reg] = (allowed_r >> (4 * L.g + reg)) & 1u;
            al4[reg] = (unsigned)__shfl((int)allowed_r, 4 * L.g + reg);
        }
#pragma unroll
        for (int t = 0; t < 4; ++t) {
            f4 pT[2], dsT[2], ds[2], pd[2];
            float delta[2];
            {
                f4 sT[2] = {f4_zero(), f4_zero()};
#pragma unroll
                for (int kk = 0; kk < 2; ++kk) {
                    sT[0] = dvs_mfma(k[t][kk], q[t][kk], sT[0]);
                    sT[1] = dvs_mfma(k[t][kk + 2], q[t][kk + 2], sT[1]);
                }
                float m[2], den[2];
#pragma unroll
                for (int u = 0; u < 2; ++u) {
                    float mx = -3.0e38f;
#pragma unroll
                    for (int reg = 0; reg < 4; ++reg) mx = ok[reg] ? fmaxf(mx, sT[u][reg]) : mx;
                    m[u] = mx;
                }
#pragma unroll
                for (int u = 0; u < 2; ++u) m[u] = dvs_max_x16(m[u]);
#pragma unroll
                for (int u = 0; u < 2; ++u) m[u] = dvs_max_x32(m[u]);
#pragma unroll
                for (int u = 0; u < 2; ++u) {
                    float sum = 0.f;
#pragma unroll
                    for (int reg = 0; reg < 4; ++reg) {
                        pT[u][reg] = ok[reg] ? __expf(sT[u][reg] - m[u]) : 0.f;
                        sum += pT[u][reg];
                    }
                    den[u] = sum;
                }
#pragma unroll
                for (int u = 0; u < 2; ++u) den[u] = dvs_add_x16(den[u]);
#pragma unroll
                for (int u = 0; u < 2; ++u) den[u] = dvs_add_x32(den[u]);
#pragma unroll
                for (int u = 0; u < 2; ++u) pT[u] *= dvs_rcp(den[u]);
            }
            {
                f4 mk[2], dpT[2];
#pragma unroll
                for (int u = 0; u < 2; ++u) {
                    mk[u] = mask_T(pm, 2 * t + u, D);
                    dpT[u] = f4_zero();
                }
                {
                    f4 oa = f4_zero(), ob = f4_zero();
#pragma unroll
                    for (int kk = 0; kk < 4; ++kk) {
                        oa = dvs_mfma(pT[0][kk] * mk[0][kk], v[t][kk], oa);
                        ob = dvs_mfma(pT[1][kk] * mk[1][kk], v[t][kk], ob);
                    }
                    dvs_bf16* po = (dvs_bf16*)sB + (4 * L.g) * DVS_PLD + 16 * t + L.r;
#pragma unroll
                    for (int reg = 0; reg < 4; ++reg) {
                        dvs_bf16 oh, ol;
                        dvs_split1(hsel ? ob[reg] : oa[reg], oh, ol);
                        po[reg * DVS_PLD] = oh;
                        po[DVS_PKB + reg * DVS_PLD] = ol;
                    }
                }
#pragma unroll
// ... 93 lines not shown
```

dags_vae_search_amd/csrc/dvs_kernels.h:

```cpp
#pragma once
#include "dvs_device.h"
#include "dvs_host.h"
#include "dvs_stage.h"

#ifndef DVS_EMU
typedef hipStream_t dvs_stream_t;
#else
typedef void* dvs_stream_t;
#endif

struct DvsLN {
    const float* stats;
    const float* g;
    const float* b;
};

struct PackArgs {
    int B, N, C;
    const float* lab1h;
    const float* pos1h;
    const float* adj;
    const uint8_t* tmask;
    DvsRecord* rec;
    int* status;
};

struct EmbedArgs {
    DvsDims dims;
    const DvsRecord* rec;
    const float *W1, *W2, *lab_w, *lab_b;
    const float* embimg;
    float* out;
    int site;
    float* out2;
    int site2;
    const float* gout;
    float* slab;
    int64_t P;
    int64_t oW1, oW2, olab_w, olab_b;
};

struct AttnArgs {
    DvsDims dims;
    const DvsRecord* rec;
    const float* xin;
    DvsLN ln;
    const float* kv;
    const float *in_w, *in_b, *out_w, *out_b;
    const void* wimg;
    float* out_pre;
    float* out_stats;
    int site_prob, site_post;
    float* qkv;
};

struct FfnArgs {
    DvsDims dims;
    const float* xin;
    DvsLN ln;
    const float *l1_w, *l1_b, *l2_w, *l2_b;
    const void* wimg;
    float* out_pre;
    float* out_stats;
    float* out_norm;
    const float *ng, *nb;
    int site_hidden, site_post;
};

struct LatentArgs {
    DvsDims dims;
    const float* xenc;
    const float *fc1_w, *fc1_b, *fc2_w, *fc2_b, *fc3_w, *fc3_b;
    const float* limg;
    const float* eps_in;
    float *mu, *logvar, *z, *epsv;
    float* mem;
    float* dag_loss;
};

struct LossArgs {
    DvsDims dims;
    const DvsRecord* rec;
    const float* xin;
    DvsLN ln;
    const float *node0_w, *node0_b, *node2_w, *node2_b, *edge0_w, *edge0_b, *edge2_w, *edge2_b;
    const void* wimg;
    float* dag_loss;
    const float* gcoef;
    float* gout;
    float* slab;
    int64_t P;
    int64_t o_node0_w, o_node0_b, o_node2_w, o_node2_b, o_edge0_w, o_edge0_b, o_edge2_w, o_edge2_b, o_ln_g, o_ln_b;
};

struct FinalizeArgs {
    int B;
    float beta;
    const float* dag_loss;
    int* status;
    float* losses;
    float* host_tail;
    uint32_t host_seq;
};

struct BuildArgs {
    int B, N, C;
    const uint8_t* labels;
    const uint16_t* preds;
    DvsRecord* rec;
    int* status;
};
void dvs_launch_build_records(const BuildArgs& a, dvs_stream_t st);
void dvs_launch_pack(const PackArgs& a, dvs_stream_t st);
void dvs_launch_embed_fwd(const EmbedArgs& a, int grid, int nw, dvs_stream_t st);
enum { DVS_FPH_ATTN = 0, DVS_FPH_FFN = 1, DVS_FPH_LATENT = 2 };
#define DVS_FWD_STACK_PHASES 9
struct FwdPhase {
    int kind, pad;
    union {
        AttnArgs a;
        FfnArgs f;
        LatentArgs l;
    } u;
};
struct FwdStackArgs {
    int nphase, pad;
    FwdPhase ph[DVS_FWD_STACK_PHASES];
    DvsStagePlan plan[DVS_FWD_STACK_PHASES];
};
static_assert(sizeof(FwdStackArgs) <= 4096, "kernel argument block limit");
void dvs_launch_fwd_stack(const FwdStackArgs& s, int tag, int grid, int nw, dvs_stream_t st);
void dvs_launch_attn_fwd(const AttnArgs& a, int grid, int nw, dvs_stream_t st);
void dvs_launch_ffn_fwd(const FfnArgs& a, int grid, int nw, dvs_stream_t st);
void dvs_launch_latent_fwd(const LatentArgs& a, dvs_stream_t st);
void dvs_launch_loss_fwd(const LossArgs& a, int grid, int nw, dvs_stream_t st);
void dvs_launch_finalize(const FinalizeArgs& a, dvs_stream_t st);
void dvs_launch_unfrag(const float* frag, float* out, int B, dvs_stream_t st);

void dvs_prof_begin(const char* name, dvs_stream_t st);
void dvs_prof_end(dvs_stream_t st);
void dvs_note_hip_error(const char* what, int hip_error, const char* hip_message);
#define DVS_LAUNCH_AS(name, kernel, grid, block, lds, st, ...)                                 \
    do {                                                                                       \
        dvs_prof_begin(name, st);                                                              \
        hipLaunchKernelGGL(kernel, grid, block, lds, st, __VA_ARGS__);                         \
        const hipError_t dvs_le_ = hipGetLastError();                                          \
        if (dvs_le_ != hipSuccess) dvs_note_hip_error(name, (int)dvs_le_, hipGetErrorString(dvs_le_)); \
        dvs_prof_end(st);                                                                      \
    } while (0)
#define DVS_LAUNCH(kernel, grid, block, lds, st, ...) DVS_LAUNCH_AS(#kernel, kernel, grid, block, lds, st, __VA_ARGS__)

#ifndef DVS_EMU
#define DVS_SET_LDS(kernel, bytes)                                                                                   \
    do {                                                                                                             \
        static size_t dvs_lds_set_[16] = {0};                                                                        \
        int dvs_dev_ = 0;                                                                                            \
        if (hipGetDevice(&dvs_dev_) != hipSuccess) dvs_dev_ = -1;                                                    \
        if (dvs_dev_ < 0 || dvs_dev_ >= 16 || dvs_lds_set_[dvs_dev_] < (size_t)(bytes)) {                            \
            const hipError_t dvs_ae_ = hipFuncSetAttribute((const void*)kernel,                                      \
                                                           hipFuncAttributeMaxDynamicSharedMemorySize, (int)(bytes)); \
            if (dvs_ae_ != hipSuccess)                                                                               \
                dvs_note_hip_error("hipFuncSetAttribute(" #kernel ", max dynamic LDS)", (int)dvs_ae_,               \
                                   hipGetErrorString(dvs_ae_));                                                      \
            else if (dvs_dev_ >= 0 && dvs_dev_ < 16)                                                                 \
                dvs_lds_set_[dvs_dev_] = (size_t)(bytes);                                                            \
        }                                                                                                            \
    } while (0)
#else
#define DVS_SET_LDS(kernel, bytes) ((void)0)
#endif

struct DvsTile {
    int dag, tok0, Nl;
};
__device__ __forceinline__ DvsTile dvs_tile_of(int tile, const DvsDims& d) {
    DvsTile t;
    if (d.NT == 1) {
        t.dag = tile;
        t.tok0 = 0;
        t.Nl = d.N;
    } else {
        t.dag = tile / d.NT;
        t.tok0 = 16 * (tile - t.dag * d.NT);
        const int nl = d.N - t.tok0;
        t.Nl = nl < 0 ? 0 : (nl > 16 ? 16 : nl);
    }
    return t;
}

__device__ __forceinline__ DvsDrop dvs_drop_of(const DvsDims& d) {
    DvsDrop D;
    D.thr16 = d.drop.thr16;
    D.scale = d.drop.scale;
    D.on = d.drop.on;
    return D;
}

struct DvsRawX {
    f4 raw[4];
    float mean, rs;
};
__device__ __forceinline__ void dvs_load_x_issue(DvsRawX& r, const float* xin, const DvsLN& ln, size_t dag, const Lane& L) {
    dvs_load_tile(r.raw, xin, dag, L);
    r.mean = 0.f;
    r.rs = 1.f;
    if (ln.stats != nullptr) {
        r.mean = ln.stats[dag * 32 + L.r];
        r.rs = ln.stats[dag * 32 + 16 + L.r];
    }
}
template <bool WANT_XHAT>
__device__ __forceinline__ void dvs_load_x_finish(f4 (&x)[4], f4 (&xhat)[4], float& rstd, const DvsRawX& r, const DvsLN& ln,
                                                  const float* lg, const float* lb, int N, const Lane& L) {
    const float vm = L.r < N ? 1.f : 0.f;
// ... 86 lines not shown
```

dags_vae_search_amd/csrc/k_backward.hip:

```cpp
#include "dvs_bwd_phases.h"
#include "dvs_latent_bwd.h"

template <int NW>
__global__ __launch_bounds__(64 * NW) void k_ffn_bwd(FfnBwdArgs a, DvsStagePlan plan) {
    DVS_DYN_LDS(smem);
    dvs_ffn_bwd_phase<NW>(a, smem, &plan, true, &plan, false);
}
void dvs_launch_ffn_bwd(const FfnBwdArgs& a, int grid, int nw, dvs_stream_t st) {
    const size_t lds = ffnb_lds_bytes();
    DvsStagePlan plan;
    ffnb_plan(plan, a, DVS_FAKE_LDS);
    if (nw == 4) {
        DVS_SET_LDS(k_ffn_bwd<4>, lds);
        DVS_LAUNCH_AS("k_ffn_bwd", k_ffn_bwd<4>, dim3(grid), dim3(256), lds, st, a, plan);
    } else {
        DVS_SET_LDS(k_ffn_bwd<8>, lds);
        DVS_LAUNCH_AS("k_ffn_bwd", k_ffn_bwd<8>, dim3(grid), dim3(512), lds, st, a, plan);
    }
}

template <int NPROJ, int NW>
__global__ __launch_bounds__(64 * NW) void k_proj_bwd(ProjBwdArgs a, DvsStagePlan plan) {
    DVS_DYN_LDS(smem);
    dvs_proj_bwd_phase<NPROJ, NW>(a, smem, &plan, true, &plan, false);
}

#define DVS_PROJ_LAUNCH(NP, NWV)                                                               \
    do {                                                                                       \
        DVS_SET_LDS((k_proj_bwd<NP, NWV>), bytes);                                             \
        DVS_LAUNCH_AS("k_proj_bwd<" #NP ">", (k_proj_bwd<NP, NWV>), dim3(grid), dim3(64 * NWV), bytes, st, a, plan); \
    } while (0)
void dvs_launch_proj_bwd(const ProjBwdArgs& a, int nproj, int grid, int nw, dvs_stream_t st) {
    const size_t bytes = projb_lds_bytes(nproj);
    DvsStagePlan plan;
    projb_plan(plan, a, nproj, DVS_FAKE_LDS);
    if (nw == 4) {
        if (nproj == 3) DVS_PROJ_LAUNCH(3, 4);
        else if (nproj == 2) DVS_PROJ_LAUNCH(2, 4);
        else DVS_PROJ_LAUNCH(1, 4);
    } else {
        if (nproj == 3) DVS_PROJ_LAUNCH(3, 8);
        else if (nproj == 2) DVS_PROJ_LAUNCH(2, 8);
        else DVS_PROJ_LAUNCH(1, 8);
    }
}

template <int NW>
__global__ __launch_bounds__(64 * NW) void k_attn_bwd(AttnBwdArgs a, DvsStagePlan plan) {
    DVS_DYN_LDS(smem);
    dvs_attn_bwd_phase<NW>(a, smem, &plan, true, &plan, false);
}

void dvs_launch_attn_bwd(const AttnBwdArgs& a, int grid, int nw, dvs_stream_t st) {
    const size_t lds = attnb_lds_floats() * 4;
    DvsStagePlan plan;
    attnb_plan(plan, a, DVS_FAKE_LDS);
    if (nw == 4) {
        DVS_SET_LDS(k_attn_bwd<4>, lds);
        DVS_LAUNCH_AS("k_attn_bwd", k_attn_bwd<4>, dim3(grid), dim3(256), lds, st, a, plan);
    } else {
        DVS_SET_LDS(k_attn_bwd<8>, lds);
        DVS_LAUNCH_AS("k_attn_bwd", k_attn_bwd<8>, dim3(grid), dim3(512), lds, st, a, plan);
    }
}

template <int TAG, int NW>
__global__ __launch_bounds__(64 * NW) void k_bwd_stack(BwdStackArgs s) {
    DVS_DYN_LDS(smem);
#ifndef DVS_EMU
    const DvsPlanK plans =
        ((const __attribute__((address_space(4))) BwdStackArgs*)__builtin_amdgcn_kernarg_segment_ptr())->plan;
#else
    const DvsPlanK plans = s.plan;
#endif
    if (TAG == 1 && NW == 8 && s.has_latent) {
        const int step = (int)gridDim.x * 8, B = s.lat.dims.B;
        for (int base = dvs_bid() * 8; base < B; base += 2 * step) {
            dvs_latent_bwd_group<8>(s.lat, (f4 (*)[2][64])smem, base, base + step);
            __syncthreads();
        }
    }
    for (int i = 0; i < s.nphase; ++i) {
        const BwdPhase& ph = s.ph[i];
        const bool first = i == 0;
        const bool more = i + 1 < s.nphase;
        const DvsPlanK mine = plans + i;
        const DvsPlanK next = plans + (more ? i + 1 : i);
        switch (ph.kind) {
            case DVS_PH_FFN: dvs_ffn_bwd_phase<NW>(ph.u.f, smem, mine, first, next, more); break;
            case DVS_PH_ATTN: dvs_attn_bwd_phase<NW>(ph.u.a, smem, mine, first, next, more); break;
            case DVS_PH_PROJ1: dvs_proj_bwd_phase<1, NW>(ph.u.p, smem, mine, first, next, more); break;
            case DVS_PH_PROJ2: dvs_proj_bwd_phase<2, NW>(ph.u.p, smem, mine, first, next, more); break;
            default: dvs_proj_bwd_phase<3, NW>(ph.u.p, smem, mine, first, next, more); break;
        }
    }
}

void dvs_launch_bwd_stack(const BwdStackArgs& s_in, int tag, int grid, int nw, dvs_stream_t st) {
    BwdStackArgs s = s_in;
    for (int i = 0; i < s.nphase; ++i) {
        dvs_bwd_plan(s.plan[i], s.ph[i], DVS_FAKE_LDS);
        s.plan[i].phase = i;
    }
#ifdef DVS_STAMPS
    static int stamp_seq = 0;
    for (int i = 0; i < s.nphase; ++i) s.plan[i].phase = (stamp_seq % 3) * DVS_STACK_PHASES + i;
    ++stamp_seq;
#endif
    size_t lds = 0;
    for (int i = 0; i < s.nphase; ++i) {
        const int k = s.ph[i].kind;
        const size_t b = k == DVS_PH_FFN ? ffnb_lds_bytes() : k == DVS_PH_ATTN ? attnb_lds_floats() * 4 : projb_lds_bytes(k - DVS_PH_PROJ1 + 1);
        lds = b > lds ? b : lds;
    }
#define DVS_BSTACK_LAUNCH(TG, NWV)                                                             \
    do {                                                                                       \
        DVS_SET_LDS((k_bwd_stack<TG, NWV>), lds);                                              \
        DVS_LAUNCH_AS("k_bwd_stack<" #TG ">", (k_bwd_stack<TG, NWV>), dim3(grid), dim3(64 * NWV), lds, st, s); \
    } while (0)
    if (nw == 4) {
        if (tag == 0) DVS_BSTACK_LAUNCH(0, 4);
        else DVS_BSTACK_LAUNCH(1, 4);
    } else {
        if (tag == 0) DVS_BSTACK_LAUNCH(0, 8);
        else DVS_BSTACK_LAUNCH(1, 8);
    }
}

__global__ __launch_bounds__(256) void k_reduce_slabs(ReduceArgs a) {
    __shared__ f4 part[4][64];
    const int q = threadIdx.x >> 6, c = threadIdx.x & 63;
    const int64_t i4 = ((int64_t)blockIdx.x * 64 + c) * 4;
    const bool in = i4 < a.P;
    f4 s = f4_zero();
    if (in) {
        const bool fc = (i4 >= a.fc_lo1 && i4 < a.fc_hi1) || (i4 >= a.fc_lo2 && i4 < a.fc_hi2);
        const float* src = fc ? a.fcpart : a.slab;
        const int n = fc ? DVS_FC_PARTS : a.nslab;
        const int per = (n + 3) / 4;
        const int k1 = (q + 1) * per < n ? (q + 1) * per : n;
        int k = q * per;
        for (; k + 8 <= k1; k += 8) {
            f4 v[8];
#pragma unroll
            for (int u = 0; u < 8; ++u) v[u] = *(const f4*)(src + (size_t)(k + u) * a.P + i4);
#pragma unroll
            for (int u = 0; u < 8; ++u) s += v[u];
        }
        for (; k < k1; ++k) s += *(const f4*)(src + (size_t)k * a.P + i4);
    }
    part[q][c] = s;
    __syncthreads();
    if (q == 0) {
        const f4 tot = (part[0][c] + part[1][c]) + (part[2][c] + part[3][c]);
        if (in) *(f4*)(a.grads + i4) = tot;
        if (a.sqpart) {
            float ss = 0.f;
#pragma unroll
            for (int e = 0; e < 4; ++e) ss += (in && i4 + e < a.P) ? tot[e] * tot[e] : 0.f;
            ss = dvs_sum_wave(ss);
            if (c == 0) a.sqpart[blockIdx.x] = ss;
        }
    }
}

void dvs_launch_reduce_slabs(const ReduceArgs& a, dvs_stream_t st) {
    const int64_t n4 = (a.P + 3) / 4;
    DVS_LAUNCH(k_reduce_slabs, dim3((unsigned)((n4 + 63) / 64)), dim3(256), 0, st, a);
}

#ifdef DVS_STAMPS
DVS_STAMP_READER(bwd)
#endif
```

dags_vae_search_amd/csrc/k_forward.hip:

```cpp
#include "dvs_kernels.h"
#include "dvs_wimg.h"

constexpr int PACK_DAGS = 4;
__device__ __forceinline__ void pack_stream(float* dst, const float* __restrict__ src, size_t nfloats) {
    const size_t n4 = nfloats >> 2;
    size_t i = threadIdx.x;
    for (; i + 3 * blockDim.x < n4; i += 4 * blockDim.x) {
        f4 v[4];
#pragma unroll
        for (int u = 0; u < 4; ++u) v[u] = *(const f4*)(src + 4 * (i + u * blockDim.x));
#pragma unroll
        for (int u = 0; u < 4; ++u) *(f4*)(dst + 4 * (i + u * blockDim.x)) = v[u];
    }
    for (; i < n4; i += blockDim.x) *(f4*)(dst + 4 * i) = *(const f4*)(src + 4 * i);
    for (size_t i = 4 * n4 + threadIdx.x; i < nfloats; i += blockDim.x) dst[i] = src[i];
}
__global__ __launch_bounds__(8 * 16 * PACK_DAGS) void k_pack(PackArgs a) {
    DVS_DYN_LDS(smem);
    const int N = a.N, C = a.C;
    const int dag0 = blockIdx.x * PACK_DAGS;
    const int nd = (a.B - dag0 < PACK_DAGS) ? a.B - dag0 : PACK_DAGS;
    float* s_lab = (float*)smem;
    float* s_pos = s_lab + PACK_DAGS * 16 * 16;
    float* s_adj = s_pos + PACK_DAGS * 16 * 16;
// ... 168 lines not shown
    float *W1, *W2, *labw, *labb, *scr;
};
__device__ __forceinline__ EmbLds emb_lds(char* smem) {
    EmbLds l;
    l.W1 = (float*)smem;
    l.W2 = l.W1 + 2 * DVS_MAXTOK * DVS_LD;
    l.labw = l.W2 + 64 * EMB_LDW2;
    l.labb = l.labw + 32 * 16;
    l.scr = l.labb + 32;
    return l;
}
static size_t emb_lds_floats(int nwaves) {
    const size_t n = 2 * DVS_MAXTOK * DVS_LD + 64 * EMB_LDW2 + 32 * 16 + 32 + (size_t)nwaves * 16;
    return n > (size_t)DvsEmbImg::FLOATS ? n : (size_t)DvsEmbImg::FLOATS;
}

__global__ __launch_bounds__(1024) void k_embed_fwd(EmbedArgs a, DvsStagePlan plan) {
    DVS_DYN_LDS(smem);
    const int N = a.dims.N, C = a.dims.C;
    const EmbLds l = emb_lds(smem);
    if (blockDim.x >= 1024) dvs_stage_now<2>(&plan, smem);
    else dvs_stage_now<5>(&plan, smem);
    __syncthreads();
    const Lane L = dvs_lane();
    const DvsDrop D = dvs_drop_of(a.dims);
    float* scr = l.scr + L.wave * 16;
    for (int dag = blockIdx.x * L.nwaves + L.wave; dag < a.dims.B; dag += gridDim.x * L.nwaves) {
        const DvsRecord* rec = a.rec + dag;
        const bool valid = L.r < N;
        const EmbSel sel = dvs_emb_selectors(rec, N, scr, L);
        f4 eh[4];
        dvs_emb_hidden(eh, l.W1, N, sel, L);
        const uint32_t gdag = a.dims.dag_offset + dag;
        const int label = rec->label[L.r];
        for (int v = 0; v < (a.out2 ? 2 : 1); ++v) {
            const int site = v ? a.site2 : a.site;
            f4 e1[4];
#pragma unroll
            for (int t = 0; t < 4; ++t) e1[t] = eh[t];
            dvs_dropout_tile(e1, dvs_site_key(a.dims.seed_lo, a.dims.seed_hi, site, gdag), D, L);
            f4 x[4];
            f4 e2[2] = {f4_zero(), f4_zero()};
#pragma unroll
            for (int t = 0; t < 4; ++t) {
                const f4 w0 = dvs_wcol(l.W2, EMB_LDW2, 0, t, L), w1 = dvs_wcol(l.W2, EMB_LDW2, 16, t, L);
#pragma unroll
                for (int kk = 0; kk < 4; ++kk) {
                    e2[0] = dvs_mfma(w0[kk], e1[t][kk], e2[0]);
                    e2[1] = dvs_mfma(w1[kk], e1[t][kk], e2[1]);
                }
            }
            {
                f4 tmp[2] = {e2[0], e2[1]};
                dvs_dropout_tile<2>(tmp, dvs_site_key(a.dims.seed_lo, a.dims.seed_hi, site + 1, gdag), D, L);
                x[2] = tmp[0];
                x[3] = tmp[1];
            }
#pragma unroll
            for (int t = 0; t < 2; ++t)
#pragma unroll
                for (int kk = 0; kk < 4; ++kk) {
                    const int f = 16 * t + 4 * L.g + kk;
                    x[t][kk] = valid ? fmaxf(l.labw[f * 16 + label] + l.labb[f], 0.f) : 0.f;
                }
            if (!valid) { x[2] = f4_zero(); x[3] = f4_zero(); }
            dvs_store_tile(v ? a.out2 : a.out, dag, x, L);
        }
    }
}

void dvs_launch_embed_fwd(const EmbedArgs& a, int grid, int nw, dvs_stream_t st) {
    const size_t lds = emb_lds_floats(16) * 4;
    DvsStagePlan plan;
    dvs_plan_clear(plan);
    dvs_plan_seg(plan, DVS_FAKE_LDS, DVS_FAKE_LDS, a.embimg, 2 * DvsEmbImg::FLOATS);
    dvs_plan_seal(plan);
    DVS_SET_LDS(k_embed_fwd, lds);
    DVS_LAUNCH(k_embed_fwd, dim3(grid), dim3(nw == 4 ? 256 : 1024), lds, st, a, plan);
}

#ifdef DVS_STAMPS
DVS_STAMP_DECL(dvs_stamps_fwd);
struct DvsLatTag { int phase; };
__device__ const DvsLatTag dvs_lat_tag = {6};
#define DVS_LAT_STAMP(id) DVS_STAMP(dvs_stamps_fwd, &dvs_lat_tag, id)
DVS_ACC_STAMP_DECL(dvs_stamps_attn);
#endif
#define ASTAMP(k) DVS_ACC_STAMP(dvs_stamps_attn, ast_, k)
#include "dvs_latent.h"
struct AttnLds {
    dvs_bf16 *Win, *Wout;
    float *inb, *outb, *lg, *lb;
};
DVS_HD inline AttnLds attn_lds(char* smem) {
    AttnLds l;
    l.Win = (dvs_bf16*)smem;
    l.Wout = l.Win + 3 * 192 * DVS_LDB;
    l.inb = (float*)(l.Wout + 3 * 64 * DVS_LDB);
    l.outb = l.inb + 192;
    l.lg = l.outb + 64;
    l.lb = l.lg + 64;
    return l;
}
static size_t attn_lds_bytes() { return 3 * 256 * DVS_LDB * sizeof(dvs_bf16) + (192 + 64 + 128) * sizeof(float); }

inline void attn_plan(DvsStagePlan& p, const AttnArgs& a, char* smem) {
    const AttnLds l = attn_lds(smem);
    dvs_plan_clear(p);
    dvs_plan_seg(p, smem, l.Win, (const dvs_bf16*)a.wimg + DvsAttnImg::Win, (int)(DvsAttnImg::WoutT - DvsAttnImg::Win));
    dvs_plan_vec(p, smem, l.inb, a.in_b, 192, true);
    dvs_plan_vec(p, smem, l.outb, a.out_b, 64);
    dvs_plan_vec(p, smem, l.lg, a.ln.g, a.ln.stats ? 64 : 0);
    dvs_plan_vec(p, smem, l.lb, a.ln.b, a.ln.stats ? 64 : 0);
    dvs_plan_seal(p);
}

__device__ __forceinline__ void attn_qkv(f4 (&q)[4], f4 (&k)[4], f4 (&v)[4], const Split3T& x, const Split3T& kv,
                                         const AttnLds& l, const Lane& L) {
#pragma unroll
    for (int t = 0; t < 4; ++t) {
        q[t] = dvs_vecT(l.inb, t, L);
        k[t] = dvs_vecT(l.inb + 64, t, L);
        v[t] = f4_splat(l.inb[128 + 16 * t + L.r]);
    }
    dvs_matb3<4>(q, x, l.Win, 192, 0, L);
    dvs_matb3<4>(k, kv, l.Win, 192, 64, L);
    dvs_matb3<4, true>(v, kv, l.Win, 192, 128, L);
    const float scale = 0.35355339059327373f;
#pragma unroll
    for (int t = 0; t < 4; ++t) q[t] *= scale;
}

__device__ __forceinline__ void attn_scores_T(f4 (&s)[8], const f4 (&q)[4], const f4 (&k)[4], const Lane& L) {
#pragma unroll
    for (int h = 0; h < 8; ++h) s[h] = f4_zero();
#pragma unroll
    for (int kk = 0; kk < 2; ++kk)
#pragma unroll
        for (int t = 0; t < 4; ++t) {
            s[2 * t] = dvs_mfma(k[t][kk], q[t][kk], s[2 * t]);
            s[2 * t + 1] = dvs_mfma(k[t][kk + 2], q[t][kk + 2], s[2 * t + 1]);
        }
}
__device__ __forceinline__ void attn_softmax_T(f4 (&p)[8], float (&m)[8], float (&den)[8], const f4 (&s)[8],
                                               unsigned allowed_r, const Lane& L) {
    bool ok[4];
#pragma unroll
    for (int reg = 0; reg < 4; ++reg) ok[reg] = (allowed_r >> (4 * L.g + reg)) & 1u;
#pragma unroll
    for (int h = 0; h < 8; ++h) {
        float mx = -3.0e38f;
#pragma unroll
        for (int reg = 0; reg < 4; ++reg) mx = ok[reg] ? fmaxf(mx, s[h][reg]) : mx;
        m[h] = mx;
    }
#pragma unroll
    for (int h = 0; h < 8; ++h) m[h] = dvs_max_x16(m[h]);
#pragma unroll
    for (int h = 0; h < 8; ++h) m[h] = dvs_max_x32(m[h]);
#pragma unroll
    for (int h = 0; h < 8; ++h) {
        float sum = 0.f;
#pragma unroll
        for (int reg = 0; reg < 4; ++reg) {
            p[h][reg] = ok[reg] ? __expf(s[h][reg] - m[h]) : 0.f;
            sum += p[h][reg];
        }
        den[h] = sum;
    }
#pragma unroll
    for (int h = 0; h < 8; ++h) den[h] = dvs_add_x16(den[h]);
#pragma unroll
    for (int h = 0; h < 8; ++h) den[h] = dvs_add_x32(den[h]);
#pragma unroll
    for (int h = 0; h < 8; ++h) p[h] *= (1.0f / den[h]);
}

__device__ __forceinline__ f4 attn_drop_T(f4 p, uint32_t key, int h, const DvsDrop& D, const Lane& L) {
    if (!D.on) return p;
    const uint32_t p0 = (uint32_t)((h * 16 + L.r) * 8 + 2 * L.g);
    const uint32_t h0 = dvs_draw(key, p0), h1 = dvs_draw(key, p0 + 1);
    p[0] = ((h0 & 0xFFFFu) >= D.thr16) ? p[0] * D.scale : 0.f;
    p[1] = ((h0 >> 16) >= D.thr16) ? p[1] * D.scale : 0.f;
    p[2] = ((h1 & 0xFFFFu) >= D.thr16) ? p[2] * D.scale : 0.f;
    p[3] = ((h1 >> 16) >= D.thr16) ? p[3] * D.scale : 0.f;
    return p;
}

template <class PP>
__device__ __forceinline__ void dvs_fwd_tail(PP next, bool has_next, char* smem, PP mine) {
    if (has_next) {
        DvsPrefetch<DVS_PF_FWD_TAIL> pf;
        const bool fetcher = dvs_tid() < DVS_PF_THREADS;
        if (fetcher) dvs_prefetch_issue<false>(pf, next, dvs_tid(), DVS_PF_THREADS);
        DVS_STAMP(dvs_stamps_fwd, mine, 3);
        dvs_lds_barrier();
        DVS_STAMP(dvs_stamps_fwd, mine, 4);
        if (fetcher) dvs_prefetch_commit<false>(pf, next, smem, dvs_tid(), DVS_PF_THREADS);
        DVS_STAMP(dvs_stamps_fwd, mine, 6);
    }
}

template <int NW, class PP>
__device__ __forceinline__ void dvs_attn_fwd_phase(const AttnArgs& a, char* smem, PP mine, bool stage_mine, PP next,
                                                   bool has_next) {
    const AttnLds l = attn_lds(smem);
    DVS_STAMP(dvs_stamps_fwd, mine, 0);
    if (stage_mine) {
        dvs_stage_now<(NW >= 8 ? DVS_PF_FWD : DVS_PF_FWD_TAIL)>(mine, smem);
        __syncthreads();
    }
    DVS_STAMP(dvs_stamps_fwd, mine, 1);
    const Lane L = dvs_lane();
    const DvsDrop D = dvs_drop_of(a.dims);
    const int N = a.dims.N;
#ifdef DVS_STAMPS
    unsigned long long ast_ = __builtin_amdgcn_s_memtime();
#endif
    bool gate = !stage_mine;
    for (int base = dvs_bid() * L.nwaves; base < a.dims.B; base += gridDim.x * L.nwaves) {
        const int dag = base + L.wave;
        if (dag >= a.dims.B) {
            DVS_PHASE_GATE(gate);
            continue;
        }
        ASTAMP(7);
        f4 x[4], dummy[4], kvt[4];
        float rstd;
        {
            DvsRawX rx;
            dvs_load_x_issue(rx, a.xin, a.ln, dag, L);
            if (a.kv) dvs_load_tile(kvt, a.kv, dag, L);
            DVS_PHASE_GATE(gate);
            dvs_load_x_finish<false>(x, dummy, rstd, rx, a.ln, l.lg, l.lb, N, L);
        }
#ifdef DVS_STAMPS
        asm volatile("s_waitcnt vmcnt(0)" ::: "memory");
#endif
        ASTAMP(0);
        f4 q[4], k[4], v[4];
        {
            const Split3T xs = dvs_split3_T(x);
            if (a.kv) {
                attn_qkv(q, k, v, xs, dvs_split3_T(kvt), l, L);
            } else {
                attn_qkv(q, k, v, xs, xs, l, L);
            }
        }
        ASTAMP(1);
        const unsigned allowed_r = a.rec[dag].allowed[L.r];
        const uint32_t gdag = a.dims.dag_offset + dag;
        const uint32_t kprob = dvs_site_key(a.dims.seed_lo, a.dims.seed_hi, a.site_prob, gdag);
        f4 s[8], p[8];
        float m[8], den[8];
        attn_scores_T(s, q, k, L);
        attn_softmax_T(p, m, den, s, allowed_r, L);
        ASTAMP(2);
#pragma unroll
        for (int h = 0; h < 8; ++h) p[h] = attn_drop_T(p[h], kprob, h, D, L);
        ASTAMP(3);
        f4 o[4];
        {
            f4 oa[4], ob[4];
#pragma unroll
            for (int t = 0; t < 4; ++t) oa[t] = ob[t] = f4_zero();
#pragma unroll
            for (int kk = 0; kk < 4; ++kk)
#pragma unroll
                for (int t = 0; t < 4; ++t) {
                    oa[t] = dvs_mfma(v[t][kk], p[2 * t][kk], oa[t]);
                    ob[t] = dvs_mfma(v[t][kk], p[2 * t + 1][kk], ob[t]);
                }
#pragma unroll
            for (int t = 0; t < 4; ++t) o[t] = f4{oa[t][0], oa[t][1], ob[t][2], ob[t][3]};
        }
        ASTAMP(4);
        f4 y[4];
#pragma unroll
        for (int t = 0; t < 4; ++t) y[t] = dvs_vecT(l.outb, t, L);
        dvs_matb3<4>(y, dvs_split3_T(o), l.Wout, 64, 0, L);
        ASTAMP(5);
        dvs_dropout_tile(y, dvs_site_key(a.dims.seed_lo, a.dims.seed_hi, a.site_post, gdag), D, L);
        const bool valid = L.r < N;
#pragma unroll
        for (int t = 0; t < 4; ++t)
#pragma unroll
            for (int kk = 0; kk < 4; ++kk) y[t][kk] = valid ? x[t][kk] + y[t][kk] : 0.f;
        dvs_store_pre(a.out_pre, a.out_stats, dag, y, L);
        ASTAMP(6);
    }
    DVS_PHASE_GATE(gate);
    DVS_STAMP(dvs_stamps_fwd, mine, 2);
    dvs_fwd_tail(next, has_next, smem, mine);
}

template <int NW>
__global__ __launch_bounds__(64 * NW) void k_attn_fwd(AttnArgs a, DvsStagePlan plan) {
    DVS_DYN_LDS(smem);
    dvs_attn_fwd_phase<NW>(a, smem, &plan, true, &plan, false);
}

void dvs_launch_attn_fwd(const AttnArgs& a, int grid, int nw, dvs_stream_t st) {
    const size_t lds = attn_lds_bytes();
    DvsStagePlan plan;
    attn_plan(plan, a, DVS_FAKE_LDS);
    if (nw == 4) {
        DVS_SET_LDS(k_attn_fwd<4>, lds);
        DVS_LAUNCH_AS("k_attn_fwd", k_attn_fwd<4>, dim3(grid), dim3(256), lds, st, a, plan);
    } else {
        DVS_SET_LDS(k_attn_fwd<8>, lds);
        DVS_LAUNCH_AS("k_attn_fwd", k_attn_fwd<8>, dim3(grid), dim3(512), lds, st, a, plan);
    }
}

struct FfnLds {
    dvs_bf16 *W1, *W2;
    float *b1, *b2, *lg, *lb, *ng, *nb;
};
DVS_HD inline FfnLds ffn_lds(char* smem) {
    FfnLds l;
    l.W1 = (dvs_bf16*)smem;
    l.W2 = l.W1 + 3 * 64 * DVS_LDB;
    l.b1 = (float*)(l.W2 + 3 * 64 * DVS_LDB);
    l.b2 = l.b1 + 64;
    l.lg = l.b2 + 64;
    l.lb = l.lg + 64;
    l.ng = l.lb + 64;
    l.nb = l.ng + 64;
    return l;
}
static size_t ffn_lds_bytes() { return 6 * 64 * DVS_LDB * sizeof(dvs_bf16) + 6 * 64 * sizeof(float); }

inline void ffn_plan(DvsStagePlan& p, const FfnArgs& a, char* smem) {
    const FfnLds l = ffn_lds(smem);
    dvs_plan_clear(p);
    dvs_plan_seg(p, smem, l.W1, (const dvs_bf16*)a.wimg + DvsFfnImg::W1, (int)(6 * DVS_IMG64));
    dvs_plan_vec(p, smem, l.b1, a.l1_b, 64);
    dvs_plan_vec(p, smem, l.b2, a.l2_b, 64);
    dvs_plan_vec(p, smem, l.lg, a.ln.g, a.ln.stats ? 64 : 0);
    dvs_plan_vec(p, smem, l.lb, a.ln.b, a.ln.stats ? 64 : 0);
    dvs_plan_vec(p, smem, l.ng, a.ng, a.out_norm ? 64 : 0);
    dvs_plan_vec(p, smem, l.nb, a.nb, a.out_norm ? 64 : 0);
    dvs_plan_seal(p);
}

template <class PP>
__device__ __forceinline__ void dvs_ffn_fwd_phase(const FfnArgs& a, char* smem, PP mine, bool stage_mine, PP next,
                                                  bool has_next) {
    const FfnLds l = ffn_lds(smem);
    DVS_STAMP(dvs_stamps_fwd, mine, 0);
    if (stage_mine) {
        dvs_stage_now<DVS_PF_FWD>(mine, smem);
        __syncthreads();
    }
    DVS_STAMP(dvs_stamps_fwd, mine, 1);
    const Lane L = dvs_lane();
    const DvsDrop D = dvs_drop_of(a.dims);
    const int ntiles = a.dims.B * a.dims.NT;
    bool gate = !stage_mine;
    for (int base = dvs_bid() * L.nwaves; base < ntiles; base += gridDim.x * L.nwaves) {
        const int tile = base + L.wave;
        if (tile >= ntiles) {
            DVS_PHASE_GATE(gate);
            continue;
        }
        const DvsTile T = dvs_tile_of(tile, a.dims);
        f4 x[4], dummy[4];
        float rstd;
        {
            DvsRawX rx;
            dvs_load_x_issue(rx, a.xin, a.ln, tile, L);
            DVS_PHASE_GATE(gate);
            dvs_load_x_finish<false>(x, dummy, rstd, rx, a.ln, l.lg, l.lb, T.Nl, L);
        }
        const uint32_t gdag = a.dims.dag_offset + T.dag;
        f4 h[4];
#pragma unroll
        for (int t = 0; t < 4; ++t) h[t] = dvs_vecT(l.b1, t, L);
        dvs_matb3<4>(h, dvs_split3_T(x), l.W1, 64, 0, L);
#pragma unroll
        for (int t = 0; t < 4; ++t)
#pragma unroll
            for (int kk = 0; kk < 4; ++kk) h[t][kk] = fmaxf(h[t][kk], 0.f);
        dvs_dropout_tile(h, dvs_site_key(a.dims.seed_lo, a.dims.seed_hi, a.site_hidden, gdag), D, L, T.tok0);
        f4 y[4];
#pragma unroll
        for (int t = 0; t < 4; ++t) y[t] = dvs_vecT(l.b2, t, L);
        dvs_matb3<4>(y, dvs_split3_T(h), l.W2, 64, 0, L);
        dvs_dropout_tile(y, dvs_site_key(a.dims.seed_lo, a.dims.seed_hi, a.site_post, gdag), D, L, T.tok0);
        const bool valid = L.r < T.Nl;
#pragma unroll
        for (int t = 0; t < 4; ++t)
#pragma unroll
            for (int kk = 0; kk < 4; ++kk) y[t][kk] = valid ? x[t][kk] + y[t][kk] : 0.f;
        float mean, rs;
        dvs_ln_stats(y, mean, rs);
        dvs_store_tile(a.out_pre, tile, y, L);
        if (L.g == 0) {
            a.out_stats[(size_t)tile * 32 + L.r] = mean;
            a.out_stats[(size_t)tile * 32 + 16 + L.r] = rs;
        }
        if (a.out_norm) {
            f4 xn[4];
#pragma unroll
            for (int t = 0; t < 4; ++t) {
                const f4 g = dvs_vecT(l.ng, t, L), b = dvs_vecT(l.nb, t, L);
#pragma unroll
                for (int kk = 0; kk < 4; ++kk) xn[t][kk] = valid ? (y[t][kk] - mean) * rs * g[kk] + b[kk] : 0.f;
            }
            dvs_store_tile(a.out_norm, tile, xn, L);
        }
    }
    DVS_PHASE_GATE(gate);
    DVS_STAMP(dvs_stamps_fwd, mine, 2);
    dvs_fwd_tail(next, has_next, smem, mine);
}

__global__ __launch_bounds__(1024) void k_ffn_fwd(FfnArgs a, DvsStagePlan plan) {
    DVS_DYN_LDS(smem);
    dvs_ffn_fwd_phase(a, smem, &plan, true, &plan, false);
}

void dvs_launch_ffn_fwd(const FfnArgs& a, int grid, int nw, dvs_stream_t st) {
    const size_t lds = ffn_lds_bytes();
    DvsStagePlan plan;
    ffn_plan(plan, a, DVS_FAKE_LDS);
    DVS_SET_LDS(k_ffn_fwd, lds);
    DVS_LAUNCH(k_ffn_fwd, dim3(grid), dim3(nw == 4 ? 256 : 1024), lds, st, a, plan);
}

template <int TAG, int NW>
__global__ __launch_bounds__(64 * NW) void k_fwd_stack(FwdStackArgs s) {
    DVS_DYN_LDS(smem);
#ifndef DVS_EMU
    const DvsPlanK plans =
        ((const __attribute__((address_space(4))) FwdStackArgs*)__builtin_amdgcn_kernarg_segment_ptr())->plan;
#else
    const DvsPlanK plans = s.plan;
#endif
    for (int i = 0; i < s.nphase; ++i) {
        const FwdPhase& ph = s.ph[i];
        const bool first = i == 0, more = i + 1 < s.nphase;
        const DvsPlanK mine = plans + i;
        if (TAG == 0 && NW == 8 && ph.kind == DVS_FPH_LATENT) {
            const int step = (int)gridDim.x * 8, B = ph.u.l.dims.B;
            for (int base = dvs_bid() * 8; base < B; base += 2 * step) {
                __syncthreads();
                dvs_latent_fwd_group(ph.u.l, smem, base, base + step);
            }
            continue;
        }
        const bool more_img = more && s.ph[i + 1].kind != DVS_FPH_LATENT;
        const DvsPlanK next = plans + (more_img ? i + 1 : i);
        if (ph.kind == DVS_FPH_ATTN) dvs_attn_fwd_phase<NW>(ph.u.a, smem, mine, first, next, more_img);
        else dvs_ffn_fwd_phase(ph.u.f, smem, mine, first, next, more_img);
    }
}

void dvs_launch_fwd_stack(const FwdStackArgs& s_in, int tag, int grid, int nw, dvs_stream_t st) {
    FwdStackArgs s = s_in;
    for (int i = 0; i < s.nphase; ++i) {
        if (s.ph[i].kind == DVS_FPH_ATTN) attn_plan(s.plan[i], s.ph[i].u.a, DVS_FAKE_LDS);
        else if (s.ph[i].kind == DVS_FPH_FFN) ffn_plan(s.plan[i], s.ph[i].u.f, DVS_FAKE_LDS);
        else dvs_plan_clear(s.plan[i]);
        s.plan[i].phase = i;
    }
#ifdef DVS_STAMPS
    for (int i = 0; i < s.nphase; ++i) s.plan[i].phase = tag * DVS_FWD_STACK_PHASES + i;
#endif
    const size_t la = attn_lds_bytes(), lf = ffn_lds_bytes();
    const size_t lds = la > lf ? la : lf;
#define DVS_FSTACK_LAUNCH(TG, NWV)                                                             \
    do {                                                                                       \
        DVS_SET_LDS((k_fwd_stack<TG, NWV>), lds);                                              \
        DVS_LAUNCH_AS("k_fwd_stack<" #TG ">", (k_fwd_stack<TG, NWV>), dim3(grid), dim3(64 * NWV), lds, st, s); \
    } while (0)
    if (nw == 4) {
        if (tag == 0) DVS_FSTACK_LAUNCH(0, 4);
        else DVS_FSTACK_LAUNCH(1, 4);
    } else {
        if (tag == 0) DVS_FSTACK_LAUNCH(0, 8);
        else DVS_FSTACK_LAUNCH(1, 8);
    }
}

__global__ void k_unfrag(const float* frag, float* out, int B) {
    const size_t i = (size_t)blockIdx.x * blockDim.x + threadIdx.x;
    if (i >= (size_t)B * 1024) return;
    const size_t dag = i >> 10;
    const int e = (int)(i & 1023);
    const int t = e >> 8, lane = (e >> 2) & 63, kk = e & 3;
    const int r = lane & 15, g = lane >> 4;
    out[dag * 1024 + r * 64 + 16 * t + 4 * g + kk] = frag[i];
}
void dvs_launch_unfrag(const float* frag, float* out, int B, dvs_stream_t st) {
    const size_t n = (size_t)B * 1024;
    DVS_LAUNCH(k_unfrag, dim3((unsigned)((n + 255) / 256)), dim3(256), 0, st, frag, out, B);
}

#ifdef DVS_STAMPS
DVS_STAMP_READER(attn)
DVS_STAMP_READER(fwd)
#endif
```

include/dvs.h:

```cpp
#ifndef DVS_H
#define DVS_H

#include <stddef.h>
#include <stdint.h>

#ifdef __cplusplus
extern "C" {
#endif

#define DVS_VERSION 202
#define DVS_NUM_PARAMS 108
#define DVS_RECORD_BYTES 96
#define DVS_RECORD_BYTES_WIDE 864
#define DVS_CLIP_SCRATCH_FLOATS 4096
#define DVS_DECODE_STATE_BYTES 440

typedef struct dvs_shape {
    int32_t batch;
    int32_t n_tokens;
    int32_t n_classes;
    int32_t training;
    float dropout;
    float beta;
    float eps_scale;
// ... 70 lines not shown

#define DVS_STRUCT_HASH_INVALID 0x7fffffffffffffffull
int dvs_decoded_structures(int32_t batch, int32_t n_vars, int32_t preds_are_u64, const void* states, size_t state_bytes,
                           uint64_t hash_mask, uint8_t* flags, uint8_t* labels, void* preds, uint64_t* keys,
                           size_t keys_bytes, uint64_t* hashes, void* stream);

int dvs_structset_filter(int32_t batch, int32_t n_vars, const uint64_t* sorted_hashes, const int64_t* order,
                         const uint64_t* keys, size_t keys_bytes, const uint8_t* flags, int32_t seen_count,
                         const uint64_t* seen_hashes, const uint64_t* seen_keys, size_t seen_keys_bytes, uint8_t* out,
                         void* stream);

#define DVS_GEN_LABELS_CHOICE 1
#define DVS_GEN_ACCEPT_ISOLATES 2
#define DVS_GEN_ACCEPT_NO_CONNECTIVITY 4
#define DVS_GEN_GROUP_SHIFT 8
int dvs_generate_dags(int32_t batch, int32_t n_vars, int32_t card, int32_t preds_are_u64, const int32_t* num_edges,
                      uint64_t seed, int64_t dag_offset, int32_t try_limit, int32_t flags, uint8_t* labels, void* preds,
                      size_t preds_bytes, int32_t* attempts, void* stream);

int dvs_generate_edge_counts(int32_t batch, int32_t n_entries, const int32_t* edge_counts, const int32_t* cum_weights,
                             uint64_t seed, int64_t dag_offset, int32_t* num_edges, void* stream);

int dvs_bic_scores(int32_t batch, int32_t n_vars, int32_t n_samples, const uint64_t* data, const uint8_t* card,
                   const uint64_t* parents, double* scratch, double* out, int32_t* status, void* stream);

typedef enum dvs_score_type {
    DVS_SCORE_LOGLIK = 0,
    DVS_SCORE_AIC = 1,
    DVS_SCORE_BIC = 2,
    DVS_SCORE_BDE = 3,
    DVS_SCORE_BDS = 4,
    DVS_SCORE_K2 = 5,
    DVS_SCORE_BDJ = 6
} dvs_score_type;
int dvs_bn_scores(int32_t batch, int32_t n_vars, int32_t n_samples, const uint64_t* data, const uint8_t* card,
                  const uint64_t* parents, int32_t score_type, double score_arg, double* scratch, double* out,
                  int32_t* status, void* stream);

int dvs_bn_toggle_scores(int32_t batch, int32_t n_vars, int32_t n_samples, const uint64_t* data, const uint8_t* card,
                         const uint64_t* parents, int32_t score_type, double score_arg, const int32_t* worklist,
                         double* local, size_t local_bytes, double* toggles, size_t toggles_bytes, int32_t* status,
                         void* stream);

int dvs_hc_step(int32_t batch, int32_t n_vars, uint64_t* parents, double* local, const double* toggles, size_t toggles_bytes,
                int32_t max_parents, double min_delta, const uint64_t* forbidden, int32_t step_cap, int32_t* worklist,
                int32_t* steps, int32_t* converged, int32_t* flags, int64_t* trace, size_t trace_bytes, int32_t* active,
                void* stream);

int dvs_tabu_step(int32_t batch, int32_t n_vars, uint64_t* parents, double* local, const double* toggles, size_t toggles_bytes,
                  int32_t max_parents, double min_delta, const uint64_t* forbidden, int32_t step_cap, int32_t* worklist,
                  int32_t* steps, int32_t* converged, int32_t* flags, int64_t* trace, size_t trace_bytes, int32_t* active,
                  int32_t tabu_len, uint64_t* ring, size_t ring_bytes, int32_t* visited, int32_t max_stall, int32_t* stall,
                  double* best_score, uint64_t* best_parents, size_t best_bytes, void* stream);

int dvs_hc_perturb(int32_t batch, int32_t n_vars, uint64_t* parents, double* local, const double* toggles, size_t toggles_bytes,
                   int32_t max_parents, const uint64_t* forbidden, int32_t* worklist, int32_t* flags, uint64_t seed,
                   uint32_t draw_index, void* stream);

int dvs_bic_parent_masks(int32_t batch, int32_t n_vars, int32_t preds_are_u64, const uint8_t* labels, const void* preds,
                         uint64_t* parents, int32_t* status, void* stream);

int dvs_gp_predict(int32_t batch, int32_t n_inducing, int32_t dim, const float* x, const float* inducing,
                   const double* alpha, double outputscale, double lengthscale, double constant, double* out,
                   void* stream);

int dvs_gp_kernel(int32_t na, int32_t nb, int32_t dim, const float* xa, const float* xb, double outputscale,
                  double lengthscale, double* K, void* stream);
int dvs_gp_kernel_backward(int32_t na, int32_t nb, int32_t dim, int32_t symmetric, const float* xa, const float* xb,
                           double outputscale, double lengthscale, const double* G, double* dxa, double* row_sums,
                           void* stream);

#define DVS_GP_ACQ_MAX_INDUCING 1023
int dvs_gp_acquire(int32_t batch, int32_t n_inducing, int32_t dim, int32_t ld, const float* x, const float* inducing,
                   const double* weights, double c0, double outputscale, double lengthscale, double constant, double best,
                   double xi, double* mean, double* var, double* ei, float* grad, void* stream);

void dvs_profile_enable(int on);
int dvs_profile_collect(char* names, int name_stride, int* counts, float* total_ms, int cap);

int dvs_debug_launch(size_t dynamic_lds_bytes, void* stream);

int dvs_debug_activation(const dvs_shape* s, const void* workspace, int slot, float* out, void* stream);

#ifdef __cplusplus
}
#endif
#endif
```

Baseline: 3.452 million DAGs/s.

## Move fwd/bwd phase tables to cached device memory and merge stacks into single chains

Replaces the kernel-argument phase stacks, which were split into several launches by a small per-launch phase limit, with one device-resident phase table per direction. The table is uploaded through a cache keyed on its contents, and per-step seeds and offsets are stripped from it so it can be reused across steps. Encoder and decoder forward now run as a single persistent chain kernel, and backward runs as one chain with the latent step inlined. The goal is fewer launches and less kernel-argument traffic, at the cost of reading phase arguments from global memory and a host upload whenever the table changes.

```diff
diff --git a/dags_vae_search_amd/_lib.py b/dags_vae_search_amd/_lib.py
--- a/dags_vae_search_amd/_lib.py
+++ b/dags_vae_search_amd/_lib.py
@@ -127,12 +127,15 @@
     lib.dvs_profile_collect.argtypes = [c_void_p, c_int, c_void_p, c_void_p, c_int]
     lib.dvs_debug_activation.restype = c_int
     lib.dvs_debug_activation.argtypes = [P(DvsShape), c_void_p, c_int, c_void_p, c_void_p]
+    lib.dvs_debug_table_stats.restype = None
+    lib.dvs_debug_table_stats.argtypes = [c_void_p, c_void_p]
     return lib
 
 
 EXPORTS = ["dvs_version", "dvs_last_error", "dvs_device_cus", "dvs_param_count", "dvs_param_table",
            "dvs_workspace_bytes", "dvs_record_bytes", "dvs_pack_features", "dvs_build_records", "dvs_loss_forward", "dvs_loss_forward_notify", "dvs_loss_backward", "dvs_loss_backward_sq", "dvs_encode", "dvs_decode", "dvs_match_decoded", "dvs_decoded_structures", "dvs_structset_filter", "dvs_generate_dags", "dvs_generate_edge_counts", "dvs_bic_scores", "dvs_bn_scores", "dvs_bn_toggle_scores", "dvs_hc_step", "dvs_tabu_step", "dvs_hc_perturb", "dvs_bic_parent_masks", "dvs_gp_predict", "dvs_gp_kernel", "dvs_gp_kernel_backward", "dvs_gp_acquire",
-           "dvs_clip_adam", "dvs_clip_adam_from_partials", "dvs_debug_activation", "dvs_debug_launch", "dvs_profile_enable", "dvs_profile_collect"]
+           "dvs_clip_adam", "dvs_clip_adam_from_partials", "dvs_debug_activation", "dvs_debug_launch", "dvs_profile_enable", "dvs_profile_collect",
+           "dvs_debug_table_stats"]
 
 
 def profile_collect(lib):
diff --git a/dags_vae_search_amd/csrc/dvs_api.hip b/dags_vae_search_amd/csrc/dvs_api.hip
--- a/dags_vae_search_amd/csrc/dvs_api.hip
+++ b/dags_vae_search_amd/csrc/dvs_api.hip
@@ -9,6 +9,7 @@
 #include "dvs_wide.h"
 #include "dvs_wimg.h"
 #include "dvs_decode.h"
+#include "dvs_table_cache.h"
 
 static thread_local char g_err[256] = "";
 
@@ -317,15 +318,61 @@
     const char* v = getenv(name);
     return v && atoi(v) != 0;
 }
-static bool split_stack() {
-    static const bool on = env_on("DVS_SPLIT_STACK");
-    return on;
-}
-static bool latent_kernels_off() {
-    static const bool on = env_on("DVS_LATENT_KERNELS");
-    return on;
-}
+static bool split_stack() { return env_on("DVS_SPLIT_STACK"); }
+static bool latent_kernels_off() { return env_on("DVS_LATENT_KERNELS"); }
 static bool latent_in_chain(bool chain, int nw) { return chain && !latent_kernels_off() && nw == 8; }
+
+namespace {
+#ifndef DVS_EMU
+void* tb_alloc_device(size_t n) {
+    void* p = nullptr;
+    return hipMalloc(&p, n) == hipSuccess ? p : nullptr;
+}
+void* tb_alloc_staging(size_t n) {
+    void* p = nullptr;
+    return hipHostMalloc(&p, n, hipHostMallocDefault) == hipSuccess ? p : nullptr;
+}
+void tb_free_device(void* p) { (void)hipFree(p); }
+void tb_free_staging(void* p) { (void)hipHostFree(p); }
+int tb_upload(void* dev, void* staging, const void* src, size_t n, void* stream, void** fence) {
+    hipEvent_t ev = (hipEvent_t)*fence;
+    if (ev) {
+        if (hipEventSynchronize(ev) != hipSuccess) return 1;
+    } else {
+        if (hipEventCreateWithFlags(&ev, hipEventDisableTiming) != hipSuccess) return 1;
+        *fence = (void*)ev;
+    }
+    memcpy(staging, src, n);
+    if (hipMemcpyAsync(dev, staging, n, hipMemcpyHostToDevice, (hipStream_t)stream) != hipSuccess) return 2;
+    return hipEventRecord(ev, (hipStream_t)stream) == hipSuccess ? 0 : 3;
+}
+void tb_free_fence(void* fence) { (void)hipEventDestroy((hipEvent_t)fence); }
+int tb_device() {
+    int dev = 0;
+    return hipGetDevice(&dev) == hipSuccess ? dev : -1;
+}
+#else
+void* tb_alloc_device(size_t n) { return malloc(n); }
+void* tb_alloc_staging(size_t n) { return malloc(n); }
+void tb_free_device(void* p) { free(p); }
+void tb_free_staging(void* p) { free(p); }
+int tb_upload(void* dev, void* staging, const void* src, size_t n, void*, void**) {
+    memcpy(staging, src, n);
+    memcpy(dev, staging, n);
+    return 0;
+}
+void tb_free_fence(void*) {}
+int tb_device() { return 0; }
+#endif
+const DvsTableBackend g_table_backend = {tb_alloc_device, tb_alloc_staging, tb_free_device, tb_free_staging, tb_upload, tb_free_fence};
+DvsTableCache g_tables;
+}
+extern "C" void dvs_debug_table_stats(int64_t* rebuilds, int64_t* lookups) {
+    if (rebuilds) *rebuilds = g_tables.rebuilds();
+    if (lookups) *lookups = g_tables.lookups();
+}
+static DvsKeys keys_of(const DvsDims& d) { return DvsKeys{d.seed_lo, d.seed_hi, d.dag_offset}; }
+static void strip_keys(DvsDims& d) { d.seed_lo = d.seed_hi = d.dag_offset = 0; }
 
 struct FwdGrids {
     int chain;
@@ -686,37 +733,72 @@
     else dvs_launch_loss_fwd(a, c.g.tiles8, 8, c.st);
 }
 struct FwdChain {
-    FwdStackArgs stack;
+    FwdChainTable table;
+    FwdChainCall call;
+    int nphase = 0;
+    int cut = -1;
     const Step& c;
-    int tag;
     bool chain;
-    FwdChain(const Step& step, int tag_) : c(step), tag(tag_), chain(!step.wide && !split_stack()) { memset(&stack, 0, sizeof(stack)); }
-    FwdPhase& next(int kind) {
-        if (stack.nphase == DVS_FWD_STACK_PHASES) flush();
-        FwdPhase& ph = stack.ph[stack.nphase++];
+    int kind;
+    explicit FwdChain(const Step& step, int table_kind = DVS_TABLE_FWD) : c(step), chain(!step.wide && !split_stack()), kind(table_kind) {
+        memset(&table, 0, sizeof(table));
+        memset(&call, 0, sizeof(call));
+        call.keys = keys_of(step.d);
+        call.lat_at = -1;
+    }
+    FwdPhase* next(int kind) {
+        if (nphase == DVS_FWD_CHAIN_PHASES) {
+            dvs_note_hip_error("forward chain", -1, "more than DVS_FWD_CHAIN_PHASES phases (launcher bug)");
+            return nullptr;
+        }
+        FwdPhase& ph = table.ph[nphase++];
         ph.kind = kind;
-        return ph;
+        return &ph;
     }
     void attn(const AttnArgs& a) {
-        if (chain) next(DVS_FPH_ATTN).u.a = a;
-        else launch_attn_fwd(c, a);
+        if (!chain) return launch_attn_fwd(c, a);
+        if (FwdPhase* ph = next(DVS_FPH_ATTN)) {
+            ph->u.a = a;
+            strip_keys(ph->u.a.dims);
+        }
     }
     void ffn(const FfnArgs& f) {
-        if (chain) next(DVS_FPH_FFN).u.f = f;
-        else launch_ffn_fwd(c, f);
-    }
-    bool latent(const LatentArgs& l) {
-        if (!latent_in_chain(chain, c.nw) || stack.nphase == 0 || stack.nphase == DVS_FWD_STACK_PHASES) return false;
-        next(DVS_FPH_LATENT).u.l = l;
-        return true;
-    }
-    void flush() {
-        if (stack.nphase > 0) dvs_launch_fwd_stack(stack, tag, c.g.chain, c.nw, c.st);
-        stack.nphase = 0;
+        if (!chain) return launch_ffn_fwd(c, f);
+        if (FwdPhase* ph = next(DVS_FPH_FFN)) {
+            ph->u.f = f;
+            strip_keys(ph->u.f.dims);
+        }
+    }
+    void latent(const LatentArgs& l) {
+        if (!chain) return dvs_launch_latent_fwd(l, c.st);
+        call.lat = l;
+        if (latent_in_chain(chain, c.nw)) call.lat_at = nphase;
+        else cut = nphase;
+    }
+    void finish() {
+        if (!chain || (nphase == 0 && cut < 0)) return;
+        const size_t lds = dvs_fwd_chain_prepare(table, nphase);
+        DvsTableCache::Use use(g_tables, g_table_backend, tb_device(), (void*)c.st, kind, &table, sizeof(table));
+        const FwdChainTable* dev = (const FwdChainTable*)use.ptr();
+        if (!dev) return dvs_note_hip_error("forward phase table", -1, "device allocation or upload failed");
+        auto run = [&](int p0, int p1) {
+            if (p0 >= p1 && !(call.lat_at >= p0 && call.lat_at <= p1)) return;
+            FwdChainCall cm = call;
+            cm.p0 = p0;
+            cm.p1 = p1;
+            dvs_launch_fwd_chain(dev, cm, lds, c.g.chain, c.nw, c.st);
+        };
+        if (cut < 0) {
+            run(0, nphase);
+        } else {
+            run(0, cut);
+            dvs_launch_latent_fwd(call.lat, c.st);
+            run(cut, nphase);
+        }
     }
 };
 
-static void encoder_forward(const Step& c, const LatentArgs& lat, bool dec_embed = false, bool save_qkv = false) {
+static void encoder_forward(const Step& c, FwdChain& chain, const LatentArgs& lat, bool dec_embed = false, bool save_qkv = false) {
     EmbedArgs e = embed_args(c, 0);
     e.out = c.ws + c.W.act[0];
     if (dec_embed) {
@@ -724,7 +806,6 @@
         e.site2 = 2;
     }
     launch_embed_fwd(c, e);
-    FwdChain chain(c, 0);
     const DvsNormP* norm = nullptr;
     int prev = 0;
     for (int i = 0; i < DVS_LAYERS; ++i) {
@@ -743,13 +824,10 @@
         norm = &pl.n2;
         prev = sf;
     }
-    const bool fused = chain.latent(lat);
-    chain.flush();
-    if (!fused) dvs_launch_latent_fwd(lat, c.st);
-}
-
-static void decoder_forward(const Step& c, int dec_in) {
-    FwdChain chain(c, 1);
+    chain.latent(lat);
+}
+
+static void decoder_forward(const Step& c, FwdChain& chain, int dec_in) {
     const DvsNormP* norm = nullptr;
     int prev = dec_in;
     for (int i = 0; i < DVS_LAYERS; ++i) {
@@ -761,7 +839,6 @@
         norm = &pl.n3;
         prev = s2;
     }
-    chain.flush();
 }
 
 extern "C" int dvs_loss_forward(const dvs_shape* s, const void* records, size_t records_bytes, const float* params,
@@ -781,8 +858,12 @@
     if (int e = check_buffers(c, "dvs_loss_forward", records_bytes, n_params, workspace_bytes)) return e;
     call_begin();
     prepare_images(c);
-    encoder_forward(c, latent_args(c, eps, true), c.d.drop.on, true);
-    decoder_forward(c, c.d.drop.on ? 7 : 0);
+    {
+        FwdChain chain(c);
+        encoder_forward(c, chain, latent_args(c, eps, true), c.d.drop.on, true);
+        decoder_forward(c, chain, c.d.drop.on ? 7 : 0);
+        chain.finish();
+    }
     launch_loss_fwd(c, loss_args(c));
     FinalizeArgs fa;
     fa.B = c.d.B;
@@ -810,7 +891,11 @@
     prepare_images(c);
     LatentArgs la = latent_args(c, nullptr, false);
     la.dims.training = 0;
-    encoder_forward(c, la);
+    {
+        FwdChain chain(c, DVS_TABLE_FWD_ENCODE);
+        encoder_forward(c, chain, la);
+        chain.finish();
+    }
     const size_t nb = (size_t)c.d.B * 32 * sizeof(float);
     copy_out(mu, c.ws + c.W.mu, nb, c.st);
     copy_out(logvar, c.ws + c.W.logvar, nb, c.st);
@@ -843,7 +928,11 @@
     e.out = c.ws + c.W.act[7];
     for (int idx = 2; idx < c.d.N; ++idx) {
         launch_embed_fwd(c, e);
-        decoder_forward(c, 7);
+        {
+            FwdChain chain(c, DVS_TABLE_FWD_DECODE);
+            decoder_forward(c, chain, 7);
+            chain.finish();
+        }
         a.idx = idx;
         dvs_launch_decode_step(a, c.g.dec4, c.st);
     }
diff --git a/dags_vae_search_amd/csrc/dvs_api_backward.inc b/dags_vae_search_amd/csrc/dvs_api_backward.inc
--- a/dags_vae_search_amd/csrc/dvs_api_backward.inc
+++ b/dags_vae_search_amd/csrc/dvs_api_backward.inc
@@ -112,21 +112,40 @@
     auto flush_stack = [&]() {
         if (stack.nphase > 0) dvs_launch_bwd_stack(stack, stack_tag, grid, nw, st);
         stack.nphase = 0;
-        stack.has_latent = 0;
-    };
+    };
+    BwdChainTable table;
+    int nphase = 0;
+    if (chain) memset(&table, 0, sizeof(table));
+    BwdPhase overflow;
     auto next_phase = [&](int kind) -> BwdPhase& {
+        if (chain) {
+            if (nphase == DVS_BWD_CHAIN_PHASES) {
+                dvs_note_hip_error("backward chain", -1, "more than DVS_BWD_CHAIN_PHASES phases (launcher bug)");
+                return overflow;
+            }
+            BwdPhase& ph = table.ph[nphase++];
+            ph.kind = kind;
+            return ph;
+        }
         if (stack.nphase == DVS_STACK_PHASES) flush_stack();
         BwdPhase& ph = stack.ph[stack.nphase++];
         ph.kind = kind;
         return ph;
     };
     auto launch_ffn_bwd = [&](const FfnBwdArgs& f) {
-        if (chain || chain_local) next_phase(DVS_PH_FFN).u.f = f;
-        else dvs_launch_ffn_bwd(f, grid, nw, st);
+        if (chain || chain_local) {
+            FfnBwdArgs& d = next_phase(DVS_PH_FFN).u.f;
+            d = f;
+            if (chain) strip_keys(d.dims);
+        } else {
+            dvs_launch_ffn_bwd(f, grid, nw, st);
+        }
     };
     auto launch_attn_bwd = [&](const AttnBwdArgs& a) {
         if (chain) {
-            next_phase(DVS_PH_ATTN).u.a = a;
+            AttnBwdArgs& d = next_phase(DVS_PH_ATTN).u.a;
+            d = a;
+            strip_keys(d.dims);
         } else if (wide) {
             flush_stack();
             dvs_launch_attn_bwd_w(a, grid, st);
@@ -135,8 +154,13 @@
         }
     };
     auto launch_proj_bwd = [&](const ProjBwdArgs& a) {
-        if (chain || chain_local) next_phase(DVS_PH_PROJ1 + 2).u.p = a;
-        else dvs_launch_proj_bwd(a, 3, grid, nw, st);
+        if (chain || chain_local) {
+            ProjBwdArgs& d = next_phase(DVS_PH_PROJ1 + 2).u.p;
+            d = a;
+            if (chain) strip_keys(d.dims);
+        } else {
+            dvs_launch_proj_bwd(a, 3, grid, nw, st);
+        }
     };
 
     float* cur = ws + W.gA;
@@ -183,9 +207,14 @@
     stack_tag = 1;
     float* gdec_emb = cur;
     float* freebuf = oth;
+    const int dec_phases = nphase;
 
     const bool fc_deferred = latent_in_chain(chain, nw);
     FcDwArgs fcdw;
+    BwdChainCall call;
+    memset(&call, 0, sizeof(call));
+    call.keys = keys_of(c.d);
+    call.lat_at = -1;
     {
         LatentBwdArgs a;
         memset(&a, 0, sizeof(a));
@@ -198,12 +227,9 @@
         a.gcoef = gcoef;
         a.gz = ws + W.gz;
         a.genc = ws + W.genc;
-        if (fc_deferred) {
-            stack.has_latent = 1;
-            stack.lat = a;
-        } else {
-            dvs_launch_latent_bwd(a, st);
-        }
+        call.lat = a;
+        if (fc_deferred) call.lat_at = dec_phases;
+        else if (!chain) dvs_launch_latent_bwd(a, st);
         FcDwArgs& f = fcdw;
         memset(&f, 0, sizeof(f));
         f.dims = c.d;
@@ -219,7 +245,7 @@
         f.o_fc2_b = L.fc2_b;
         f.o_fc3_w = L.fc3_w;
         f.o_fc3_b = L.fc3_b;
-        if (!fc_deferred) dvs_launch_fc_dw(f, st);
+        if (!chain) dvs_launch_fc_dw(f, st);
     }
     cur = ws + W.genc;
     oth = freebuf;
@@ -242,7 +268,30 @@
         std::swap(cur, oth);
     }
     flush_stack();
-    if (fc_deferred) dvs_launch_fc_dw(fcdw, st);
+    if (chain) {
+        const size_t lds = dvs_bwd_chain_prepare(table, nphase);
+        DvsTableCache::Use use(g_tables, g_table_backend, tb_device(), (void*)st, DVS_TABLE_BWD, &table, sizeof(table));
+        const BwdChainTable* dev = (const BwdChainTable*)use.ptr();
+        if (!dev) {
+            dvs_note_hip_error("backward phase table", -1, "device allocation or upload failed");
+            return call_end("dvs_loss_backward");
+        }
+        if (fc_deferred) {
+            call.p0 = 0;
+            call.p1 = nphase;
+            dvs_launch_bwd_chain(dev, call, lds, grid, nw, st);
+            dvs_launch_fc_dw(fcdw, st);
+        } else {
+            call.p0 = 0;
+            call.p1 = dec_phases;
+            dvs_launch_bwd_chain(dev, call, lds, grid, nw, st);
+            dvs_launch_latent_bwd(call.lat, st);
+            dvs_launch_fc_dw(fcdw, st);
+            call.p0 = dec_phases;
+            call.p1 = nphase;
+            dvs_launch_bwd_chain(dev, call, lds, grid, nw, st);
+        }
+    }
     {
         EmbedArgs e = embed_args(c, 0);
         e.gout = cur;
diff --git a/dags_vae_search_amd/csrc/dvs_backward.h b/dags_vae_search_amd/csrc/dvs_backward.h
--- a/dags_vae_search_amd/csrc/dvs_backward.h
+++ b/dags_vae_search_amd/csrc/dvs_backward.h
@@ -86,7 +86,6 @@
 };
 
 enum { DVS_PH_FFN = 0, DVS_PH_ATTN = 1, DVS_PH_PROJ1 = 2, DVS_PH_PROJ2 = 3, DVS_PH_PROJ3 = 4 };
-#define DVS_STACK_PHASES 9
 struct BwdPhase {
     int kind, pad;
     union {
@@ -95,15 +94,28 @@
         ProjBwdArgs p;
     } u;
 };
+#define DVS_STACK_PHASES 4
 struct BwdStackArgs {
-    int nphase;
-    int has_latent;
+    int nphase, pad;
     BwdPhase ph[DVS_STACK_PHASES];
     DvsStagePlan plan[DVS_STACK_PHASES];
-    LatentBwdArgs lat;
 };
 static_assert(sizeof(BwdStackArgs) <= 4096, "kernel argument block limit");
 void dvs_launch_bwd_stack(const BwdStackArgs& s, int tag, int grid, int nw, dvs_stream_t st);
+
+#define DVS_BWD_CHAIN_PHASES 24
+struct BwdChainTable {
+    BwdPhase ph[DVS_BWD_CHAIN_PHASES];
+    DvsStagePlan plan[DVS_BWD_CHAIN_PHASES];
+};
+struct BwdChainCall {
+    DvsKeys keys;
+    int p0, p1;
+    int lat_at;
+    LatentBwdArgs lat;
+};
+size_t dvs_bwd_chain_prepare(BwdChainTable& t, int nphase);
+void dvs_launch_bwd_chain(const BwdChainTable* device_table, const BwdChainCall& cm, size_t lds, int grid, int nw, dvs_stream_t st);
 void dvs_launch_ffn_bwd(const FfnBwdArgs& a, int grid, int nw, dvs_stream_t st);
 void dvs_launch_proj_bwd(const ProjBwdArgs& a, int nproj, int grid, int nw, dvs_stream_t st);
 void dvs_launch_attn_bwd(const AttnBwdArgs& a, int grid, int nw, dvs_stream_t st);
diff --git a/dags_vae_search_amd/csrc/dvs_bwd_phases.h b/dags_vae_search_amd/csrc/dvs_bwd_phases.h
--- a/dags_vae_search_amd/csrc/dvs_bwd_phases.h
+++ b/dags_vae_search_amd/csrc/dvs_bwd_phases.h
@@ -160,7 +160,7 @@
 
 template <int NW, class PP>
 __device__ __forceinline__ void dvs_ffn_bwd_phase(const FfnBwdArgs& a, char* smem, PP mine, bool stage_mine, PP next,
-                                                  bool has_next) {
+                                                  bool has_next, const DvsKeys* call = nullptr) {
     const FfnBLds l = ffnb_lds(smem);
     DVS_STAMP(dvs_stamps_bwd, mine, 0);
     if (stage_mine) {
@@ -212,9 +212,10 @@
             dvs_wave_sync();
             dvs_ln_bwd_core(gp, pxh, prstd, l.og, L);
         }
-        const uint32_t gdag = a.dims.dag_offset + (uint32_t)T.dag;
-        const uint32_t khid = dvs_site_key(a.dims.seed_lo, a.dims.seed_hi, a.site_hidden, gdag);
-        const uint32_t kpost = dvs_site_key(a.dims.seed_lo, a.dims.seed_hi, a.site_post, gdag);
+        const DvsKeys K = dvs_keys_of(a.dims, call);
+        const uint32_t gdag = K.dag_offset + (uint32_t)T.dag;
+        const uint32_t khid = dvs_site_key(K.seed_lo, K.seed_hi, a.site_hidden, gdag);
+        const uint32_t kpost = dvs_site_key(K.seed_lo, K.seed_hi, a.site_post, gdag);
         f4 hpre[4], hd[4];
 #pragma unroll
         for (int t = 0; t < 4; ++t) hpre[t] = dvs_vecT(l.b1, t, L);
@@ -503,7 +504,7 @@
 
 template <int NW, class PP>
 __device__ __forceinline__ void dvs_attn_bwd_phase(const AttnBwdArgs& a, char* smem, PP mine, bool stage_mine, PP next,
-                                                   bool has_next) {
+                                                   bool has_next, const DvsKeys* call = nullptr) {
     const AttnBLds l = attnb_lds(smem);
     DVS_STAMP(dvs_stamps_bwd, mine, 0);
     if (stage_mine) {
@@ -528,8 +529,9 @@
         const bool live = dag < B;
         const size_t dg = live ? dag : 0;
         const int Nl = live ? N : 0;
-        const uint32_t gdag = a.dims.dag_offset + (uint32_t)dg;
-        const uint32_t kprob = dvs_site_key(a.dims.seed_lo, a.dims.seed_hi, a.site_prob, gdag);
+        const DvsKeys K = dvs_keys_of(a.dims, call);
+        const uint32_t gdag = K.dag_offset + (uint32_t)dg;
+        const uint32_t kprob = dvs_site_key(K.seed_lo, K.seed_hi, a.site_prob, gdag);
         const unsigned allowed_r = live ? a.rec[dg].allowed[L.r] : (1u << L.r);
         f4 q[4], k[4], v[4];
         {
@@ -568,7 +570,7 @@
         {
             f4 dy[4];
             dvs_load_grad(dy, a.gpre, dg, Nl, L);
-            dvs_dropout_tile(dy, dvs_site_key(a.dims.seed_lo, a.dims.seed_hi, a.site_post, gdag), D, L);
+            dvs_dropout_tile(dy, dvs_site_key(K.seed_lo, K.seed_hi, a.site_post, gdag), D, L);
             dvs_park_bf((dvs_bf16*)sA, dy, L);
 #pragma unroll
             for (int t = 0; t < 4; ++t) dOT[t] = f4_zero();
diff --git a/dags_vae_search_amd/csrc/dvs_kernels.h b/dags_vae_search_amd/csrc/dvs_kernels.h
--- a/dags_vae_search_amd/csrc/dvs_kernels.h
+++ b/dags_vae_search_amd/csrc/dvs_kernels.h
@@ -8,6 +8,14 @@
 #else
 typedef void* dvs_stream_t;
 #endif
+
+struct DvsKeys {
+    uint32_t seed_lo, seed_hi, dag_offset;
+};
+__device__ __forceinline__ DvsKeys dvs_keys_of(const DvsDims& d, const DvsKeys* call) {
+    if (call) return *call;
+    return DvsKeys{d.seed_lo, d.seed_hi, d.dag_offset};
+}
 
 struct DvsLN {
     const float* stats;
@@ -113,23 +121,27 @@
 void dvs_launch_build_records(const BuildArgs& a, dvs_stream_t st);
 void dvs_launch_pack(const PackArgs& a, dvs_stream_t st);
 void dvs_launch_embed_fwd(const EmbedArgs& a, int grid, int nw, dvs_stream_t st);
-enum { DVS_FPH_ATTN = 0, DVS_FPH_FFN = 1, DVS_FPH_LATENT = 2 };
-#define DVS_FWD_STACK_PHASES 9
+enum { DVS_FPH_ATTN = 0, DVS_FPH_FFN = 1 };
 struct FwdPhase {
     int kind, pad;
     union {
         AttnArgs a;
         FfnArgs f;
-        LatentArgs l;
     } u;
 };
-struct FwdStackArgs {
-    int nphase, pad;
-    FwdPhase ph[DVS_FWD_STACK_PHASES];
-    DvsStagePlan plan[DVS_FWD_STACK_PHASES];
-};
-static_assert(sizeof(FwdStackArgs) <= 4096, "kernel argument block limit");
-void dvs_launch_fwd_stack(const FwdStackArgs& s, int tag, int grid, int nw, dvs_stream_t st);
+#define DVS_FWD_CHAIN_PHASES 15
+struct FwdChainTable {
+    FwdPhase ph[DVS_FWD_CHAIN_PHASES];
+    DvsStagePlan plan[DVS_FWD_CHAIN_PHASES];
+};
+struct FwdChainCall {
+    DvsKeys keys;
+    int p0, p1;
+    int lat_at;
+    LatentArgs lat;
+};
+size_t dvs_fwd_chain_prepare(FwdChainTable& t, int nphase);
+void dvs_launch_fwd_chain(const FwdChainTable* device_table, const FwdChainCall& cm, size_t lds, int grid, int nw, dvs_stream_t st);
 void dvs_launch_attn_fwd(const AttnArgs& a, int grid, int nw, dvs_stream_t st);
 void dvs_launch_ffn_fwd(const FfnArgs& a, int grid, int nw, dvs_stream_t st);
 void dvs_launch_latent_fwd(const LatentArgs& a, dvs_stream_t st);
diff --git a/dags_vae_search_amd/csrc/dvs_table_cache.h b/dags_vae_search_amd/csrc/dvs_table_cache.h
--- /dev/null
+++ b/dags_vae_search_amd/csrc/dvs_table_cache.h
@@ -0,0 +1,111 @@
+#pragma once
+#include <stddef.h>
+#include <stdint.h>
+#include <string.h>
+
+#include <mutex>
+
+struct DvsTableBackend {
+    void* (*alloc_device)(size_t bytes);
+    void* (*alloc_staging)(size_t bytes);
+    void (*free_device)(void* p);
+    void (*free_staging)(void* p);
+    int (*upload)(void* dev, void* staging, const void* src, size_t bytes, void* stream, void** fence);
+    void (*free_fence)(void* fence);
+};
+
+enum { DVS_TABLE_FWD = 0, DVS_TABLE_BWD = 1, DVS_TABLE_FWD_ENCODE = 2, DVS_TABLE_FWD_DECODE = 3 };
+constexpr int DVS_TABLE_SLOTS = 16;
+
+class DvsTableCache {
+    struct Slot {
+        bool used = false;
+        int device = 0, kind = 0;
+        void* stream = nullptr;
+        size_t bytes = 0, cap = 0;
+        void* dev = nullptr;
+        void* staging = nullptr;
+        void* fence = nullptr;
+        uint64_t stamp = 0;
+    };
+    std::mutex mu_;
+    Slot slot_[DVS_TABLE_SLOTS];
+    uint64_t clock_ = 0;
+    long rebuilds_ = 0, lookups_ = 0;
+
+    void release(const DvsTableBackend& be, Slot& s, bool keep_fence = false) {
+        if (s.dev) be.free_device(s.dev);
+        if (s.staging) be.free_staging(s.staging);
+        void* const fence = s.fence;
+        if (fence && !keep_fence) be.free_fence(fence);
+        s = Slot();
+        if (keep_fence) s.fence = fence;
+    }
+    const void* get_locked(const DvsTableBackend& be, int device, void* stream, int kind, const void* src, size_t bytes) {
+        ++lookups_;
+        Slot* s = nullptr;
+        for (Slot& c : slot_)
+            if (c.used && c.device == device && c.stream == stream && c.kind == kind) s = &c;
+        if (!s) {
+            for (Slot& c : slot_)
+                if (!c.used && !s) s = &c;
+            if (!s) {
+                s = &slot_[0];
+                for (Slot& c : slot_)
+                    if (c.stamp < s->stamp) s = &c;
+                release(be, *s);
+            }
+            s->used = true;
+            s->device = device;
+            s->stream = stream;
+            s->kind = kind;
+        }
+        s->stamp = ++clock_;
+        if (s->bytes == bytes && s->dev && memcmp(s->staging, src, bytes) == 0) return s->dev;
+        if (s->cap < bytes) {
+            const Slot keep = *s;
+            release(be, *s, true);
+            s->used = true;
+            s->device = keep.device;
+            s->stream = keep.stream;
+            s->kind = keep.kind;
+            s->stamp = keep.stamp;
+            s->dev = be.alloc_device(bytes);
+            s->staging = be.alloc_staging(bytes);
+            if (!s->dev || !s->staging) {
+                release(be, *s);
+                return nullptr;
+            }
+            s->cap = bytes;
+        }
+        s->bytes = 0;
+        if (be.upload(s->dev, s->staging, src, bytes, stream, &s->fence) != 0) return nullptr;
+        s->bytes = bytes;
+        ++rebuilds_;
+        return s->dev;
+    }
+
+   public:
+    class Use {
+        std::unique_lock<std::mutex> lock_;
+        const void* ptr_;
+
+       public:
+        Use(DvsTableCache& c, const DvsTableBackend& be, int device, void* stream, int kind, const void* src, size_t bytes)
+            : lock_(c.mu_), ptr_(c.get_locked(be, device, stream, kind, src, bytes)) {}
+        const void* ptr() const { return ptr_; }
+    };
+    long rebuilds() {
+        std::lock_guard<std::mutex> g(mu_);
+        return rebuilds_;
+    }
+    long lookups() {
+        std::lock_guard<std::mutex> g(mu_);
+        return lookups_;
+    }
+    void clear(const DvsTableBackend& be) {
+        std::lock_guard<std::mutex> g(mu_);
+        for (Slot& s : slot_)
+            if (s.used) release(be, s);
+    }
+};
diff --git a/dags_vae_search_amd/csrc/k_backward.hip b/dags_vae_search_amd/csrc/k_backward.hip
--- a/dags_vae_search_amd/csrc/k_backward.hip
+++ b/dags_vae_search_amd/csrc/k_backward.hip
@@ -73,13 +73,6 @@
 #else
     const DvsPlanK plans = s.plan;
 #endif
-    if (TAG == 1 && NW == 8 && s.has_latent) {
-        const int step = (int)gridDim.x * 8, B = s.lat.dims.B;
-        for (int base = dvs_bid() * 8; base < B; base += 2 * step) {
-            dvs_latent_bwd_group<8>(s.lat, (f4 (*)[2][64])smem, base, base + step);
-            __syncthreads();
-        }
-    }
     for (int i = 0; i < s.nphase; ++i) {
         const BwdPhase& ph = s.ph[i];
         const bool first = i == 0;
@@ -102,11 +95,6 @@
         dvs_bwd_plan(s.plan[i], s.ph[i], DVS_FAKE_LDS);
         s.plan[i].phase = i;
     }
-#ifdef DVS_STAMPS
-    static int stamp_seq = 0;
-    for (int i = 0; i < s.nphase; ++i) s.plan[i].phase = (stamp_seq % 3) * DVS_STACK_PHASES + i;
-    ++stamp_seq;
-#endif
     size_t lds = 0;
     for (int i = 0; i < s.nphase; ++i) {
         const int k = s.ph[i].kind;
@@ -124,6 +112,63 @@
     } else {
         if (tag == 0) DVS_BSTACK_LAUNCH(0, 8);
         else DVS_BSTACK_LAUNCH(1, 8);
+    }
+}
+
+template <int NW>
+__global__ __launch_bounds__(64 * NW) void k_bwd_chain(const BwdChainTable* table, BwdChainCall cm) {
+    DVS_DYN_LDS(smem);
+#ifndef DVS_EMU
+    const __attribute__((address_space(4))) BwdChainTable* const tab =
+        (const __attribute__((address_space(4))) BwdChainTable*)(uintptr_t)table;
+#else
+    const BwdChainTable* const tab = table;
+#endif
+    const DvsPlanK plans = tab->plan;
+    for (int i = cm.p0; i < cm.p1; ++i) {
+        if (NW == 8 && i == cm.lat_at) {
+            __syncthreads();
+            const int step = (int)gridDim.x * 8, B = cm.lat.dims.B;
+            for (int base = dvs_bid() * 8; base < B; base += 2 * step) {
+                dvs_latent_bwd_group<8>(cm.lat, (f4 (*)[2][64])dvs_bwd_epi(smem), base, base + step);
+                __syncthreads();
+            }
+        }
+        const BwdPhase& ph = *(const BwdPhase*)&tab->ph[i];
+        const bool first = i == cm.p0;
+        const bool more = i + 1 < cm.p1;
+        const DvsPlanK mine = plans + i;
+        const DvsPlanK next = plans + (more ? i + 1 : i);
+        switch (ph.kind) {
+            case DVS_PH_FFN: dvs_ffn_bwd_phase<NW>(ph.u.f, smem, mine, first, next, more, &cm.keys); break;
+            case DVS_PH_ATTN: dvs_attn_bwd_phase<NW>(ph.u.a, smem, mine, first, next, more, &cm.keys); break;
+            case DVS_PH_PROJ1: dvs_proj_bwd_phase<1, NW>(ph.u.p, smem, mine, first, next, more); break;
+            case DVS_PH_PROJ2: dvs_proj_bwd_phase<2, NW>(ph.u.p, smem, mine, first, next, more); break;
+            default: dvs_proj_bwd_phase<3, NW>(ph.u.p, smem, mine, first, next, more); break;
+        }
+    }
+}
+
+static size_t bwd_phase_lds(int k) {
+    return k == DVS_PH_FFN ? ffnb_lds_bytes() : k == DVS_PH_ATTN ? attnb_lds_floats() * 4 : projb_lds_bytes(k - DVS_PH_PROJ1 + 1);
+}
+size_t dvs_bwd_chain_prepare(BwdChainTable& t, int nphase) {
+    size_t lds = DVS_BWD_EPI_FLOOR + sizeof(f4) * 8 * 2 * 64;
+    for (int i = 0; i < nphase; ++i) {
+        dvs_bwd_plan(t.plan[i], t.ph[i], DVS_FAKE_LDS);
+        t.plan[i].phase = i;
+        const size_t b = bwd_phase_lds(t.ph[i].kind);
+        lds = b > lds ? b : lds;
+    }
+    return lds;
+}
+void dvs_launch_bwd_chain(const BwdChainTable* table, const BwdChainCall& cm, size_t lds, int grid, int nw, dvs_stream_t st) {
+    if (nw == 4) {
+        DVS_SET_LDS(k_bwd_chain<4>, lds);
+        DVS_LAUNCH_AS("k_bwd_chain", k_bwd_chain<4>, dim3(grid), dim3(256), lds, st, table, cm);
+    } else {
+        DVS_SET_LDS(k_bwd_chain<8>, lds);
+        DVS_LAUNCH_AS("k_bwd_chain", k_bwd_chain<8>, dim3(grid), dim3(512), lds, st, table, cm);
     }
 }
 
diff --git a/dags_vae_search_amd/csrc/k_forward.hip b/dags_vae_search_amd/csrc/k_forward.hip
--- a/dags_vae_search_amd/csrc/k_forward.hip
+++ b/dags_vae_search_amd/csrc/k_forward.hip
@@ -274,7 +274,7 @@
 #ifdef DVS_STAMPS
 DVS_STAMP_DECL(dvs_stamps_fwd);
 struct DvsLatTag { int phase; };
-__device__ const DvsLatTag dvs_lat_tag = {6};
+__device__ const DvsLatTag dvs_lat_tag = {31};
 #define DVS_LAT_STAMP(id) DVS_STAMP(dvs_stamps_fwd, &dvs_lat_tag, id)
 DVS_ACC_STAMP_DECL(dvs_stamps_attn);
 #endif
@@ -395,7 +395,7 @@
 
 template <int NW, class PP>
 __device__ __forceinline__ void dvs_attn_fwd_phase(const AttnArgs& a, char* smem, PP mine, bool stage_mine, PP next,
-                                                   bool has_next) {
+                                                   bool has_next, const DvsKeys* call = nullptr) {
     const AttnLds l = attn_lds(smem);
     DVS_STAMP(dvs_stamps_fwd, mine, 0);
     if (stage_mine) {
@@ -441,8 +441,9 @@
         }
         ASTAMP(1);
         const unsigned allowed_r = a.rec[dag].allowed[L.r];
-        const uint32_t gdag = a.dims.dag_offset + dag;
-        const uint32_t kprob = dvs_site_key(a.dims.seed_lo, a.dims.seed_hi, a.site_prob, gdag);
+        const DvsKeys K = dvs_keys_of(a.dims, call);
+        const uint32_t gdag = K.dag_offset + dag;
+        const uint32_t kprob = dvs_site_key(K.seed_lo, K.seed_hi, a.site_prob, gdag);
         f4 s[8], p[8];
         float m[8], den[8];
         attn_scores_T(s, q, k, L);
@@ -472,7 +473,7 @@
         for (int t = 0; t < 4; ++t) y[t] = dvs_vecT(l.outb, t, L);
         dvs_matb3<4>(y, dvs_split3_T(o), l.Wout, 64, 0, L);
         ASTAMP(5);
-        dvs_dropout_tile(y, dvs_site_key(a.dims.seed_lo, a.dims.seed_hi, a.site_post, gdag), D, L);
+        dvs_dropout_tile(y, dvs_site_key(K.seed_lo, K.seed_hi, a.site_post, gdag), D, L);
         const bool valid = L.r < N;
 #pragma unroll
         for (int t = 0; t < 4; ++t)
@@ -538,7 +539,7 @@
 
 template <class PP>
 __device__ __forceinline__ void dvs_ffn_fwd_phase(const FfnArgs& a, char* smem, PP mine, bool stage_mine, PP next,
-                                                  bool has_next) {
+                                                  bool has_next, const DvsKeys* call = nullptr) {
     const FfnLds l = ffn_lds(smem);
     DVS_STAMP(dvs_stamps_fwd, mine, 0);
     if (stage_mine) {
@@ -565,7 +566,8 @@
             DVS_PHASE_GATE(gate);
             dvs_load_x_finish<false>(x, dummy, rstd, rx, a.ln, l.lg, l.lb, T.Nl, L);
         }
-        const uint32_t gdag = a.dims.dag_offset + T.dag;
+        const DvsKeys K = dvs_keys_of(a.dims, call);
+        const uint32_t gdag = K.dag_offset + T.dag;
         f4 h[4];
 #pragma unroll
         for (int t = 0; t < 4; ++t) h[t] = dvs_vecT(l.b1, t, L);
@@ -574,12 +576,12 @@
         for (int t = 0; t < 4; ++t)
 #pragma unroll
             for (int kk = 0; kk < 4; ++kk) h[t][kk] = fmaxf(h[t][kk], 0.f);
-        dvs_dropout_tile(h, dvs_site_key(a.dims.seed_lo, a.dims.seed_hi, a.site_hidden, gdag), D, L, T.tok0);
+        dvs_dropout_tile(h, dvs_site_key(K.seed_lo, K.seed_hi, a.site_hidden, gdag), D, L, T.tok0);
         f4 y[4];
 #pragma unroll
         for (int t = 0; t < 4; ++t) y[t] = dvs_vecT(l.b2, t, L);
         dvs_matb3<4>(y, dvs_split3_T(h), l.W2, 64, 0, L);
-        dvs_dropout_tile(y, dvs_site_key(a.dims.seed_lo, a.dims.seed_hi, a.site_post, gdag), D, L, T.tok0);
+        dvs_dropout_tile(y, dvs_site_key(K.seed_lo, K.seed_hi, a.site_post, gdag), D, L, T.tok0);
         const bool valid = L.r < T.Nl;
 #pragma unroll
         for (int t = 0; t < 4; ++t)
@@ -621,58 +623,54 @@
     DVS_LAUNCH(k_ffn_fwd, dim3(grid), dim3(nw == 4 ? 256 : 1024), lds, st, a, plan);
 }
 
-template <int TAG, int NW>
-__global__ __launch_bounds__(64 * NW) void k_fwd_stack(FwdStackArgs s) {
+template <int NW>
+__global__ __launch_bounds__(64 * NW) void k_fwd_chain(const FwdChainTable* table, FwdChainCall cm) {
     DVS_DYN_LDS(smem);
 #ifndef DVS_EMU
-    const DvsPlanK plans =
-        ((const __attribute__((address_space(4))) FwdStackArgs*)__builtin_amdgcn_kernarg_segment_ptr())->plan;
+    const __attribute__((address_space(4))) FwdChainTable* const tab =
+        (const __attribute__((address_space(4))) FwdChainTable*)(uintptr_t)table;
 #else
-    const DvsPlanK plans = s.plan;
+    const FwdChainTable* const tab = table;
 #endif
-    for (int i = 0; i < s.nphase; ++i) {
-        const FwdPhase& ph = s.ph[i];
-        const bool first = i == 0, more = i + 1 < s.nphase;
-        const DvsPlanK mine = plans + i;
-        if (TAG == 0 && NW == 8 && ph.kind == DVS_FPH_LATENT) {
-            const int step = (int)gridDim.x * 8, B = ph.u.l.dims.B;
+    const DvsPlanK plans = tab->plan;
+    bool staged = false;
+    for (int i = cm.p0;; ++i) {
+        if (NW == 8 && i == cm.lat_at) {
+            const int step = (int)gridDim.x * 8, B = cm.lat.dims.B;
             for (int base = dvs_bid() * 8; base < B; base += 2 * step) {
                 __syncthreads();
-                dvs_latent_fwd_group(ph.u.l, smem, base, base + step);
+                dvs_latent_fwd_group(cm.lat, smem, base, base + step);
             }
-            continue;
-        }
-        const bool more_img = more && s.ph[i + 1].kind != DVS_FPH_LATENT;
+            __syncthreads();
+            staged = false;
+        }
+        if (i >= cm.p1) break;
+        const FwdPhase& ph = *(const FwdPhase*)&tab->ph[i];
+        const bool more_img = i + 1 < cm.p1 && !(NW == 8 && i + 1 == cm.lat_at);
+        const DvsPlanK mine = plans + i;
         const DvsPlanK next = plans + (more_img ? i + 1 : i);
-        if (ph.kind == DVS_FPH_ATTN) dvs_attn_fwd_phase<NW>(ph.u.a, smem, mine, first, next, more_img);
-        else dvs_ffn_fwd_phase(ph.u.f, smem, mine, first, next, more_img);
-    }
-}
-
-void dvs_launch_fwd_stack(const FwdStackArgs& s_in, int tag, int grid, int nw, dvs_stream_t st) {
-    FwdStackArgs s = s_in;
-    for (int i = 0; i < s.nphase; ++i) {
-        if (s.ph[i].kind == DVS_FPH_ATTN) attn_plan(s.plan[i], s.ph[i].u.a, DVS_FAKE_LDS);
-        else if (s.ph[i].kind == DVS_FPH_FFN) ffn_plan(s.plan[i], s.ph[i].u.f, DVS_FAKE_LDS);
-        else dvs_plan_clear(s.plan[i]);
-        s.plan[i].phase = i;
-    }
-#ifdef DVS_STAMPS
-    for (int i = 0; i < s.nphase; ++i) s.plan[i].phase = tag * DVS_FWD_STACK_PHASES + i;
-#endif
+        if (ph.kind == DVS_FPH_ATTN) dvs_attn_fwd_phase<NW>(ph.u.a, smem, mine, !staged, next, more_img, &cm.keys);
+        else dvs_ffn_fwd_phase(ph.u.f, smem, mine, !staged, next, more_img, &cm.keys);
+        staged = more_img;
+    }
+}
+
+size_t dvs_fwd_chain_prepare(FwdChainTable& t, int nphase) {
+    for (int i = 0; i < nphase; ++i) {
+        if (t.ph[i].kind == DVS_FPH_ATTN) attn_plan(t.plan[i], t.ph[i].u.a, DVS_FAKE_LDS);
+        else ffn_plan(t.plan[i], t.ph[i].u.f, DVS_FAKE_LDS);
+        t.plan[i].phase = i;
+    }
     const size_t la = attn_lds_bytes(), lf = ffn_lds_bytes();
-    const size_t lds = la > lf ? la : lf;
-#define DVS_FSTACK_LAUNCH(TG, NWV)                                                             \
-    do {                                                                                       \
-        DVS_SET_LDS((k_fwd_stack<TG, NWV>), lds);                                              \
-        DVS_LAUNCH_AS("k_fwd_stack<" #TG ">", (k_fwd_stack<TG, NWV>), dim3(grid), dim3(64 * NWV), lds, st, s); \
-    } while (0)
+    return la > lf ? la : lf;
+}
+void dvs_launch_fwd_chain(const FwdChainTable* table, const FwdChainCall& cm, size_t lds, int grid, int nw, dvs_stream_t st) {
     if (nw == 4) {
-        if (tag == 0) DVS_FSTACK_LAUNCH(0, 4);
-        else DVS_FSTACK_LAUNCH(1, 4);
+        DVS_SET_LDS(k_fwd_chain<4>, lds);
+        DVS_LAUNCH_AS("k_fwd_chain", k_fwd_chain<4>, dim3(grid), dim3(256), lds, st, table, cm);
     } else {
-        if (tag == 0) DVS_FSTACK_LAUNCH(0, 8);
-        else DVS_FSTACK_LAUNCH(1, 8);
+        DVS_SET_LDS(k_fwd_chain<8>, lds);
+        DVS_LAUNCH_AS("k_fwd_chain", k_fwd_chain<8>, dim3(grid), dim3(512), lds, st, table, cm);
     }
 }
 
diff --git a/include/dvs.h b/include/dvs.h
--- a/include/dvs.h
+++ b/include/dvs.h
@@ -176,6 +176,8 @@
 
 int dvs_debug_activation(const dvs_shape* s, const void* workspace, int slot, float* out, void* stream);
 
+void dvs_debug_table_stats(int64_t* rebuilds, int64_t* lookups);
+
 #ifdef __cplusplus
 }
 #endif
```

After: 3.513 million DAGs/s (median of 6 runs). +1.8%, better.
